# actionml/universal-recommender

Hardware: AMD Instinct MI355X
Metric: cooccurrence pairs/sec (A'A+A'B) + LLR top-k items/sec (higher is better)
Workload: dtype int32 counts / f64 LLR; 1 GPU; config4: synthetic 10M users x 2M items, Zipf-1.0, 5 event types (purchase/view/add-to-cart/search/category-pref); generator=torch Philox on the GPU (universal_recommender_amd.synth.generate_device), maxEventsPerEventType=500, maxCorrelatorsPerEventType=50, seed=20260925, entry_point=urcco_context_build_device (C ABI, include/urcco.h), launch=one process per GPU, parallelism=items range-partitioned over 1 GPU(s), one HIP stream per event type

## Files before the change

universal-recommender_amd/csrc/cco_common.h:

```cpp
#pragma once
#include "cco_kernels.h"

namespace urcco {


constexpr int WAVE = 64;

__device__ __forceinline__ unsigned long long shfl_xor_u64(unsigned long long v, int m) {
  unsigned lo = (unsigned)v, hi = (unsigned)(v >> 32);
  lo = __shfl_xor(lo, m);
  hi = __shfl_xor(hi, m);
  return ((unsigned long long)hi << 32) | lo;
}
__device__ __forceinline__ long long shfl_i64(long long v, int src) {
  unsigned lo = (unsigned)v, hi = (unsigned)((unsigned long long)v >> 32);
  lo = __shfl(lo, src);
  hi = __shfl(hi, src);
  return (long long)(((unsigned long long)hi << 32) | lo);
}
__device__ __forceinline__ long long shfl_up_i64(long long v, unsigned d) {
  unsigned lo = (unsigned)v, hi = (unsigned)((unsigned long long)v >> 32);
  lo = __shfl_up(lo, d);
  hi = __shfl_up(hi, d);
  return (long long)(((unsigned long long)hi << 32) | lo);
// ... 59 lines not shown
    tot += sw;
  }
  __syncthreads();
  *total = tot;
  return base + inc - v;
}

template <typename Load>
__global__ __launch_bounds__(SCAN_THREADS) void scan_reduce_kernel(Load ld, int64_t n, int64_t* __restrict__ tile_sums,
                                                                   const int64_t* __restrict__ n_live) {
  __shared__ long long s_wave[SCAN_THREADS / WAVE];
  const int64_t base = (int64_t)blockIdx.x * SCAN_TILE;
  if (n_live && base >= *n_live) {
    if (threadIdx.x == 0) tile_sums[blockIdx.x] = 0;
    return;
  }
  long long v = 0;
#pragma unroll
  for (int q = 0; q < SCAN_ITEMS; ++q) {
    const int64_t i = base + (int64_t)q * SCAN_THREADS + threadIdx.x;
    if (i < n) v += ld(i);
  }
  long long tot;
  block_exclusive_scan(v, s_wave, &tot);
  if (threadIdx.x == 0) tile_sums[blockIdx.x] = tot;
}

constexpr int ST_THREADS = 1024;
constexpr int ST_ITEMS = 8;
static __global__ __launch_bounds__(ST_THREADS) void scan_tiles_kernel(int64_t* __restrict__ tile_sums, int64_t n_tiles, const int64_t* __restrict__ n_live,
                                                                       ExpandForm form) {
  __shared__ long long s_wave[ST_THREADS / WAVE];
  __shared__ int s_over;
  if (threadIdx.x == 0) s_over = 0;
  __syncthreads();
  bool over = false;
  const int lane = threadIdx.x & (WAVE - 1), wave = threadIdx.x / WAVE;
  int64_t live_tiles = n_tiles;
  if (n_live) {
    const int64_t lt = *n_live / SCAN_TILE + 1;
    if (lt < live_tiles) live_tiles = lt;
  }
  long long carry = form.seed;
  for (int64_t base = 0; base < live_tiles; base += ST_THREADS * ST_ITEMS) {
    const int64_t first = base + (int64_t)threadIdx.x * ST_ITEMS;
    long long x[ST_ITEMS];
    long long sum = 0;
#pragma unroll
    for (int q = 0; q < ST_ITEMS; ++q) {
      x[q] = first + q < live_tiles ? tile_sums[first + q] : 0;
      sum += x[q];
      over = over || (unsigned long long)x[q] >= form.limit;
    }
    long long inc = sum;
#pragma unroll
    for (int d = 1; d < WAVE; d <<= 1) {
      const long long o = shfl_up_i64(inc, d);
      if (lane >= d) inc += o;
    }
    if (lane == WAVE - 1) s_wave[wave] = inc;
    __syncthreads();
    long long before = 0, tot = 0;
#pragma unroll
    for (int w = 0; w < ST_THREADS / WAVE; ++w) {
      const long long sw = s_wave[w];
      if (w < wave) before += sw;
      tot += sw;
    }
    __syncthreads();
    long long run = carry + before + inc - sum;
#pragma unroll
    for (int q = 0; q < ST_ITEMS; ++q) {
      if (first + q < live_tiles) tile_sums[first + q] = run;
      run += x[q];
    }
    carry += tot;
  }
  for (int64_t t = live_tiles + threadIdx.x; t < n_tiles; t += ST_THREADS) tile_sums[t] = carry;
  if (threadIdx.x == 0) tile_sums[n_tiles] = carry;
  if (form.word) {
    if (over) s_over = 1;
    __syncthreads();
    if (threadIdx.x == 0) {
      int f = form.host_narrow ? 0 : *form.word;
      if (form.host_narrow) s_over = 0;
      if (s_over) f |= FORM_TILE;
      if (form.pack_bad && *form.pack_bad != 0) f |= FORM_PACK;
      if (form.host_wide) f |= FORM_HOST;
      *form.word = f ? (f | FORM_WIDE) : 0;
    }
  }
}

template <typename Load>
__global__ __launch_bounds__(SCAN_THREADS) void scan_downsweep_kernel(Load ld, int64_t n, const int64_t* __restrict__ tile_sums,
                                                                      int64_t n_tiles, int64_t* __restrict__ out,
                                                                      const int64_t* __restrict__ n_live) {
  __shared__ long long s_wave[SCAN_THREADS / WAVE];
  if (n_live && (int64_t)blockIdx.x * SCAN_TILE > *n_live) return;
  const int64_t first = (int64_t)blockIdx.x * SCAN_TILE + (int64_t)threadIdx.x * SCAN_ITEMS;
  static_assert(SCAN_ITEMS == 8, "load8");
  long long x[SCAN_ITEMS];
  long long v = 0;
  const bool interior = first + SCAN_ITEMS <= n;
  if (interior) {
    ld.load8(first, x);
  } else {
#pragma unroll
    for (int q = 0; q < SCAN_ITEMS; ++q) x[q] = first + q < n ? ld(first + q) : 0;
  }
#pragma unroll
  for (int q = 0; q < SCAN_ITEMS; ++q) v += x[q];
  long long tot;
  long long run = block_exclusive_scan(v, s_wave, &tot) + tile_sums[blockIdx.x];
  if (interior && (reinterpret_cast<uintptr_t>(out) & 15) == 0) {
#pragma unroll
    for (int q = 0; q < SCAN_ITEMS; q += 2) {
      const long long e0 = run, e1 = run + x[q];
      run = e1 + x[q + 1];
      int4 w;
      w.x = (int)(unsigned)e0; w.y = (int)(unsigned)((unsigned long long)e0 >> 32);
      w.z = (int)(unsigned)e1; w.w = (int)(unsigned)((unsigned long long)e1 >> 32);
      *reinterpret_cast<int4*>(out + first + q) = w;
    }
  } else {
#pragma unroll
    for (int q = 0; q < SCAN_ITEMS; ++q) {
      const int64_t i = first + q;
      if (i < n) out[i] = run;
      run += x[q];
    }
  }
  if (blockIdx.x == 0 && threadIdx.x == 0) out[n] = tile_sums[n_tiles];
}

constexpr int SB_THREADS = 1024;
constexpr int SB_ITEMS = 8;
constexpr int64_t SB_MAX = 32768;
template <typename Load>
__global__ __launch_bounds__(SB_THREADS) void scan_block_kernel(Load ld, int64_t n, int64_t* __restrict__ out) {
  __shared__ long long s_wave[SB_THREADS / WAVE];
  const int lane = threadIdx.x & (WAVE - 1), wave = threadIdx.x / WAVE;
  long long carry = 0;
  for (int64_t base = 0; base < n; base += SB_THREADS * SB_ITEMS) {
    const int64_t first = base + (int64_t)threadIdx.x * SB_ITEMS;
    long long x[SB_ITEMS];
    long long sum = 0;
    if (first + SB_ITEMS <= n) {
      ld.load8(first, x);
    } else {
#pragma unroll
      for (int q = 0; q < SB_ITEMS; ++q) x[q] = first + q < n ? ld(first + q) : 0;
    }
#pragma unroll
    for (int q = 0; q < SB_ITEMS; ++q) sum += x[q];
    long long inc = sum;
#pragma unroll
    for (int d = 1; d < WAVE; d <<= 1) {
      const long long o = shfl_up_i64(inc, d);
      if (lane >= d) inc += o;
    }
    if (lane == WAVE - 1) s_wave[wave] = inc;
    __syncthreads();
    long long before = 0, tot = 0;
#pragma unroll
    for (int w = 0; w < SB_THREADS / WAVE; ++w) {
      const long long sw = s_wave[w];
// ... 30 lines not shown
```

universal-recommender_amd/csrc/cco_counts.hip:

```cpp
#include "cco_kernels.h"

#include <atomic>
#include <cstdio>
#include <cstdlib>

#include "cco_common.h"
#include "cco_device.h"


namespace urcco {

constexpr int CC_THREADS = 256;
constexpr int CC_SLOTS = 4096;

__device__ __forceinline__ void cc_insert(int* s_key, int* s_cnt, int32_t* __restrict__ counts, int col) {
  const int key = col + 1;
  unsigned h = ((unsigned)key * 0x9E3779B1u) >> 20;
#pragma unroll
  for (int probe = 0; probe < 2; ++probe) {
    int kk = __hip_atomic_load(&s_key[h], __ATOMIC_RELAXED, __HIP_MEMORY_SCOPE_WORKGROUP);
    if (kk == 0) kk = atomicCAS(&s_key[h], 0, key), kk = (kk == 0) ? key : kk;
    if (kk == key) {
      atomicAdd(&s_cnt[h], 1);
      return;
// ... 164 lines not shown
    const long long dst = s_base[b];
    for (int t = lane; t < len; t += WAVE) bucketed[dst + t] = s_stage[l0 + t];
  }
}

__global__ __launch_bounds__(SCAN_THREADS) void ph_blockmap_kernel(const int64_t* __restrict__ offsets, int n_buckets, int64_t n_parts,
                                                                  int32_t* __restrict__ blk_prefix, int PH_CHUNK) {
  __shared__ long long s_wave[SCAN_THREADS / WAVE];
  long long carry = 0;
  for (int base = 0; base < n_buckets; base += SCAN_THREADS) {
    const int b = base + threadIdx.x;
    long long v = 0;
    if (b < n_buckets) {
      const long long size = offsets[(int64_t)(b + 1) * n_parts] - offsets[(int64_t)b * n_parts];
      v = (size + PH_CHUNK - 1) / PH_CHUNK;
    }
    long long tot;
    const long long ex = block_exclusive_scan(v, s_wave, &tot);
    if (b < n_buckets) blk_prefix[b] = (int32_t)(carry + ex);
    carry += tot;
  }
  if (threadIdx.x == 0) blk_prefix[n_buckets] = (int32_t)carry;
}

constexpr int PHH_THREADS = 1024;
__global__ __launch_bounds__(PHH_THREADS) void ph_hist_kernel(const unsigned short* __restrict__ bucketed, const int64_t* __restrict__ offsets,
                                                      int n_buckets, int64_t n_parts, const int32_t* __restrict__ blk_prefix,
                                                      unsigned short* __restrict__ partial, int PH_CHUNK) {
  __shared__ unsigned s_cnt[PH_BUCKET];
  const int blk = blockIdx.x;
  if (blk >= blk_prefix[n_buckets]) return;
  int lo = 0, hi = n_buckets;
  while (hi - lo > 1) {
    const int mid = (lo + hi) >> 1;
    if (blk_prefix[mid] <= blk) lo = mid; else hi = mid;
  }
  const int b = lo;
  for (int c = threadIdx.x; c < PH_BUCKET; c += PHH_THREADS) s_cnt[c] = 0u;
  __syncthreads();
  const int64_t bs = offsets[(int64_t)b * n_parts], be = offsets[(int64_t)(b + 1) * n_parts];
  const int64_t e0 = bs + (int64_t)(blk - blk_prefix[b]) * PH_CHUNK;
  const int64_t e1 = e0 + PH_CHUNK < be ? e0 + PH_CHUNK : be;
  int64_t e = e0 + threadIdx.x;
  const int64_t a0 = (e0 + 7) & ~(int64_t)7;
  for (; e < e1 && e < a0; e += PHH_THREADS) atomicAdd(&s_cnt[bucketed[e]], 1u);
  for (int64_t v = a0 + (int64_t)threadIdx.x * 8; v + 7 < e1; v += PHH_THREADS * 8) {
    const uint4 x = *reinterpret_cast<const uint4*>(bucketed + v);
    atomicAdd(&s_cnt[x.x & 0xffffu], 1u); atomicAdd(&s_cnt[x.x >> 16], 1u);
    atomicAdd(&s_cnt[x.y & 0xffffu], 1u); atomicAdd(&s_cnt[x.y >> 16], 1u);
    atomicAdd(&s_cnt[x.z & 0xffffu], 1u); atomicAdd(&s_cnt[x.z >> 16], 1u);
    atomicAdd(&s_cnt[x.w & 0xffffu], 1u); atomicAdd(&s_cnt[x.w >> 16], 1u);
  }
  {
    const int64_t n_vec = e1 > a0 ? (e1 - a0) / 8 : 0;
    for (int64_t t = a0 + n_vec * 8 + threadIdx.x; t < e1; t += PHH_THREADS) atomicAdd(&s_cnt[bucketed[t]], 1u);
  }
  __syncthreads();
  unsigned* out = reinterpret_cast<unsigned*>(partial + (int64_t)blk * PH_BUCKET);
  for (int c = threadIdx.x; c < PH_BUCKET / 2; c += PHH_THREADS) out[c] = s_cnt[2 * c] | (s_cnt[2 * c + 1] << 16);
}

__global__ __launch_bounds__(256) void ph_reduce_kernel(const unsigned short* __restrict__ partial, const int32_t* __restrict__ blk_prefix, int32_t n_cols,
                                                        int32_t* __restrict__ counts) {
  const int64_t j = (int64_t)blockIdx.x * 256 + threadIdx.x;
  if (j >= n_cols) return;
  const int b = (int)(j >> PH_BITS);
  const int c = (int)(j & (PH_BUCKET - 1));
  unsigned sum = 0;
  for (int blk = blk_prefix[b]; blk < blk_prefix[b + 1]; ++blk) sum += partial[(int64_t)blk * PH_BUCKET + c];
  counts[j] = (int32_t)sum;
}

constexpr int PL_BITS = 14;
constexpr int PL_BUCKET = 1 << PL_BITS;
constexpr int PL_PART = 16384;
constexpr int PL_THREADS = 512;
constexpr int PL_PER_THREAD = PL_PART / PL_THREADS;
constexpr int PL_MAX_BUCKETS = 256;
constexpr int PL_COPIES = 16;
static_assert(PL_PER_THREAD % 4 == 0 && PL_PART / PL_COPIES <= 1024 && PL_THREADS % PL_COPIES == 0, "packed word: 8 + 14 + 10 bits");

__global__ __launch_bounds__(PL_THREADS, 6) void pl_partition_kernel(const int32_t* __restrict__ ci, int64_t nnz_host, const int64_t* __restrict__ nnz_dev,
                                                                  int n_buckets, int64_t n_parts, unsigned short* __restrict__ bucketed,
                                                                  unsigned short* __restrict__ loc_t, int vec_ok) {
  __shared__ int s_cnt[PL_COPIES * PL_MAX_BUCKETS];
  __shared__ uint4 s_stage4[PL_PART / 8];
  __shared__ long long s_wave[PL_THREADS / WAVE];
  unsigned short* s_stage = reinterpret_cast<unsigned short*>(s_stage4);
  const int64_t nnz = nnz_dev ? *nnz_dev : nnz_host;
  const int64_t e0 = (int64_t)blockIdx.x * PL_PART;
  const int64_t e1 = e0 + PL_PART < nnz ? e0 + PL_PART : nnz;
  if (e0 >= e1) {
    for (int b = threadIdx.x; b <= n_buckets; b += PL_THREADS) loc_t[(int64_t)b * n_parts + blockIdx.x] = 0;
    return;
  }
  for (int b = threadIdx.x; b < PL_COPIES * n_buckets; b += PL_THREADS) s_cnt[b] = 0;
  __syncthreads();
  int* mine = s_cnt + (threadIdx.x & (PL_COPIES - 1)) * n_buckets;
  const int n = (int)(e1 - e0);
  auto live = [&](int q) { return (q >> 2) * (PL_THREADS * 4) + (int)threadIdx.x * 4 + (q & 3) < n; };
  unsigned w[PL_PER_THREAD];
#pragma unroll
  for (int r = 0; r < PL_PER_THREAD / 4; ++r) {
    const int64_t e = e0 + (int64_t)r * (PL_THREADS * 4) + (int64_t)threadIdx.x * 4;
    int4 x = make_int4(0, 0, 0, 0);
    if (vec_ok && e + 3 < e1) {
      x = *reinterpret_cast<const int4*>(ci + e);
    } else {
      if (e < e1) x.x = ci[e];
      if (e + 1 < e1) x.y = ci[e + 1];
      if (e + 2 < e1) x.z = ci[e + 2];
      if (e + 3 < e1) x.w = ci[e + 3];
    }
    w[4 * r] = (unsigned)x.x; w[4 * r + 1] = (unsigned)x.y; w[4 * r + 2] = (unsigned)x.z; w[4 * r + 3] = (unsigned)x.w;
  }
#pragma unroll
  for (int q = 0; q < PL_PER_THREAD; ++q) {
    if (live(q)) {
      const unsigned b = w[q] >> PL_BITS;
      const unsigned rank = (unsigned)atomicAdd(&mine[b], 1);
      w[q] = (b << 24) | ((w[q] & (PL_BUCKET - 1)) << 10) | rank;
    }
  }
  __syncthreads();
  {
    const int b = threadIdx.x;
    long long tot = 0;
    if (b < n_buckets) {
#pragma unroll
      for (int k = 0; k < PL_COPIES; ++k) tot += s_cnt[k * n_buckets + b];
    }
    long long all;
    const long long ex = block_exclusive_scan<PL_THREADS>(tot, s_wave, &all);
    if (b < n_buckets) {
      int run = (int)ex;
      loc_t[(int64_t)b * n_parts + blockIdx.x] = (unsigned short)run;
#pragma unroll
      for (int k = 0; k < PL_COPIES; ++k) {
        const int c = s_cnt[k * n_buckets + b];
        s_cnt[k * n_buckets + b] = run;
        run += c;
      }
    }
    if (b == n_buckets) loc_t[(int64_t)b * n_parts + blockIdx.x] = (unsigned short)all;
  }
  __syncthreads();
#pragma unroll
  for (int q = 0; q < PL_PER_THREAD; ++q) {
    if (live(q)) s_stage[mine[w[q] >> 24] + (int)(w[q] & 1023u)] = (unsigned short)((w[q] >> 10) & (PL_BUCKET - 1));
  }
  __syncthreads();
  uint4* dst = reinterpret_cast<uint4*>(bucketed + e0);
  for (int v = threadIdx.x; v * 8 < n; v += PL_THREADS) dst[v] = s_stage4[v];
}

constexpr int PLH_THREADS = 1024;
constexpr int PL_LANES = 8;
__global__ __launch_bounds__(PLH_THREADS) void pl_hist_kernel(const unsigned short* __restrict__ bucketed, const unsigned short* __restrict__ loc_t,
                                                              int n_buckets, int64_t n_parts, const int32_t* __restrict__ blk_prefix, int32_t n_cols,
                                                              unsigned* __restrict__ partial) {
  __shared__ unsigned s_cnt[PL_BUCKET];
  const int blk = blockIdx.x;
  if (blk >= blk_prefix[n_buckets]) return;
  int blo = 0, bhi = n_buckets;
  while (bhi - blo > 1) {
    const int mid = (blo + bhi) >> 1;
    if (blk_prefix[mid] <= blk) blo = mid; else bhi = mid;
  }
  const int b = blo, s = blk - blk_prefix[b], S = blk_prefix[b + 1] - blk_prefix[b];
  const int width = (int)((int64_t)n_cols - ((int64_t)b << PL_BITS) < PL_BUCKET ? (int64_t)n_cols - ((int64_t)b << PL_BITS) : PL_BUCKET);
  for (int c = threadIdx.x; c < width; c += PLH_THREADS) s_cnt[c] = 0u;
  __syncthreads();
  const int64_t pp = (n_parts + S - 1) / S;
  const int64_t p0 = (int64_t)s * pp < n_parts ? (int64_t)s * pp : n_parts, p1 = p0 + pp < n_parts ? p0 + pp : n_parts;
  const int lane = threadIdx.x & (WAVE - 1), wave = threadIdx.x / WAVE;
  const unsigned short* lo_t = loc_t + (int64_t)b * n_parts;
  const unsigned short* hi_t = loc_t + (int64_t)(b + 1) * n_parts;
  constexpr int SPR = WAVE / PL_LANES;
  constexpr int GP = 16;
  static_assert(GP % SPR == 0 && SPR <= GP, "rounds per group");
  const int sub = lane / PL_LANES, sl = lane % PL_LANES;
  const int64_t gstep = (int64_t)(PLH_THREADS / WAVE) * GP;
  int64_t g = p0 + (int64_t)wave * GP;
  unsigned lo_n = 0u, hi_n = 0u;
  if (g < p1 && lane < GP && g + lane < p1) {
    lo_n = lo_t[g + lane];
    hi_n = hi_t[g + lane];
  }
  for (; g < p1; g += gstep) {
    const unsigned lo = lo_n, hi = hi_n;
    lo_n = 0u;
    hi_n = 0u;
    if (g + gstep < p1 && lane < GP && g + gstep + lane < p1) {
      lo_n = lo_t[g + gstep + lane];
      hi_n = hi_t[g + gstep + lane];
    }
    const int rounds = (int)(p1 - g < GP ? (p1 - g + SPR - 1) / SPR : GP / SPR);
    for (int r = 0; r < rounds; ++r) {
      const int pj = SPR * r + sub;
      const unsigned lo_j = (unsigned)__shfl((int)lo, pj);
      const unsigned hi_j = (unsigned)__shfl((int)hi, pj);
      const unsigned short* src = bucketed + (g + pj) * PL_PART;
      for (unsigned base = (lo_j & ~7u) + 16u * (unsigned)sl; base < hi_j; base += 16u * PL_LANES) {
        const uint4 x0 = *reinterpret_cast<const uint4*>(src + base), x1 = *reinterpret_cast<const uint4*>(src + base + 8);
        const unsigned wds[8] = {x0.x, x0.y, x0.z, x0.w, x1.x, x1.y, x1.z, x1.w};
#pragma unroll
        for (int k = 0; k < 8; ++k) {
          const unsigned t = base + 2u * k;
          if (t >= lo_j && t < hi_j) atomicAdd(&s_cnt[wds[k] & (PL_BUCKET - 1)], 1u);
          if (t + 1u >= lo_j && t + 1u < hi_j) atomicAdd(&s_cnt[(wds[k] >> 16) & (PL_BUCKET - 1)], 1u);
        }
      }
    }
  }
  __syncthreads();
  unsigned* out = partial + (int64_t)blk * PL_BUCKET;
  for (int c = threadIdx.x; c < width; c += PLH_THREADS) out[c] = s_cnt[c];
}

__global__ __launch_bounds__(256) void pl_reduce_kernel(const unsigned* __restrict__ partial, const int32_t* __restrict__ blk_prefix, int32_t n_cols,
                                                        int32_t* __restrict__ counts) {
  const int64_t j = (int64_t)blockIdx.x * 256 + threadIdx.x;
  if (j >= n_cols) return;
  const int b = (int)(j >> PL_BITS);
  const int c = (int)(j & (PL_BUCKET - 1));
  unsigned sum = 0;
  for (int blk = blk_prefix[b]; blk < blk_prefix[b + 1]; ++blk) sum += partial[(int64_t)blk * PL_BUCKET + c];
  counts[j] = (int32_t)sum;
}

__global__ __launch_bounds__(256) void pl_weights_kernel(const unsigned short* __restrict__ loc_t, int64_t n_parts, unsigned long long* __restrict__ weight) {
  __shared__ long long s_wave[256 / WAVE];
  const unsigned short* lo_t = loc_t + (int64_t)blockIdx.x * n_parts;
  const unsigned short* hi_t = lo_t + n_parts;
  long long sum = 0;
  for (int64_t p = (int64_t)blockIdx.y * 256 + threadIdx.x; p < n_parts; p += (int64_t)gridDim.y * 256) sum += (long long)hi_t[p] - (long long)lo_t[p];
  long long tot;
  block_exclusive_scan<256>(sum, s_wave, &tot);
  if (threadIdx.x == 0 && tot != 0) atomicAdd(&weight[blockIdx.x], (unsigned long long)tot);
}
__global__ __launch_bounds__(SCAN_THREADS) void pl_blockmap_kernel(const long long* __restrict__ weight, int n_buckets, int64_t n_parts, int S,
                                                                  int32_t* __restrict__ blk_prefix) {
  __shared__ long long s_wave[SCAN_THREADS / WAVE];
  __shared__ long long s_total;
  {
    const int b = threadIdx.x;
    long long tot;
    block_exclusive_scan(b < n_buckets ? weight[b] : 0ll, s_wave, &tot);
    if (threadIdx.x == 0) s_total = tot;
  }
  __syncthreads();
  const long long total = s_total;
  const int b = threadIdx.x;
  long long v = 0;
  if (b < n_buckets) {
    v = total > 0 ? (weight[b] * (long long)S * n_buckets + total - 1) / total : 1;
    if (v < 1) v = 1;
    if (v > n_parts) v = n_parts;
  }
  long long tot;
  const long long ex = block_exclusive_scan(v, s_wave, &tot);
  if (b < n_buckets) blk_prefix[b] = (int32_t)ex;
  if (b == 0) blk_prefix[n_buckets] = (int32_t)tot;
}

constexpr int64_t PL_BLOCK_IDS = 49152;
static inline int pl_splits(int n_buckets, int64_t n_parts, bool bounded = true) {
  int64_t S = (2048 + n_buckets - 1) / n_buckets;
  if (S > n_parts / 4) S = n_parts / 4;
  if (bounded) {
    const int64_t by_work = n_parts * PL_PART / ((int64_t)n_buckets * PL_BLOCK_IDS);
    if (S > by_work) S = by_work;
  }
  if (S < 1) S = 1;
  return (int)S;
}
static inline int64_t pl_max_blocks(int n_buckets, int S) { return ((int64_t)S + 1) * n_buckets; }
static inline bool pl_fits(int32_t n_cols) { return (((int64_t)n_cols + PL_BUCKET - 1) >> PL_BITS) <= PL_MAX_BUCKETS; }
static inline bool pl_applies(int32_t n_cols) {
  const char* e = getenv("URCCO_COLCOUNT_GLOBAL_LAYOUT");
  if (e && *e == '1') return false;
  return pl_fits(n_cols);
}

hipError_t launch_slice_weights(hipStream_t st, const unsigned short* loc_t, int n_buckets, int64_t n_parts, long long* weight) {
  hipError_t we = hipMemsetAsync(weight, 0, sizeof(long long) * (size_t)n_buckets, st);
  if (we != hipSuccess) return we;
  const unsigned wsplit = (unsigned)(n_parts >= 8192 ? 8 : (n_parts >= 1024 ? 4 : 1));
  hipLaunchKernelGGL(pl_weights_kernel, dim3((unsigned)n_buckets, wsplit), dim3(256), 0, st, loc_t, n_parts, reinterpret_cast<unsigned long long*>(weight));
  return hipGetLastError();
}

int64_t column_counts_scratch_bytes(int64_t nnz, int32_t n_cols) {
  auto al = [](int64_t v) { return (v + 255) / 256 * 256; };
  if (nnz < PH_MIN_NNZ) return 0;
  int64_t need = 0;
  if (pl_fits(n_cols)) {
    const int64_t n_buckets = ((int64_t)n_cols + PL_BUCKET - 1) >> PL_BITS;
    const int64_t n_parts = (nnz + PL_PART - 1) / PL_PART;
    need = al(n_parts * PL_PART * 2 + 64) + al((n_buckets + 1) * n_parts * 2) + al(n_buckets * 8) + al((n_buckets + 1) * 4) +
           al(pl_max_blocks((int)n_buckets, pl_splits((int)n_buckets, n_parts, false)) * (int64_t)PL_BUCKET * 4);
  }
  if ((((int64_t)n_cols + PH_BUCKET - 1) >> PH_BITS) <= PH_MAX_BUCKETS) {
    const int64_t n_buckets = ((int64_t)n_cols + PH_BUCKET - 1) >> PH_BITS;
    const int64_t n_parts = (nnz + PH_PART - 1) / PH_PART;
    const int64_t m = n_buckets * n_parts;
    const int64_t max_blocks = n_buckets + (nnz + PH_CHUNK_SMALL - 1) / PH_CHUNK_SMALL;
    const int64_t ph = al(m * 4) + al((m + 1) * 8) + al(((m + SCAN_TILE - 1) / SCAN_TILE + 2) * 8) + al(nnz * 2 + 16) + al((n_buckets + 1) * 4) + al(max_blocks * PH_BUCKET * 2);
    if (ph > need) need = ph;
  }
  return need;
}

hipError_t launch_column_counts_partitioned(hipStream_t st, const int32_t* col_idx, int64_t nnz, const int64_t* nnz_dev, int32_t n_cols,
                                            int32_t* counts, char* scratch) {
  auto al = [](int64_t v) { return (v + 255) / 256 * 256; };
  const int vec_ok = (reinterpret_cast<uintptr_t>(col_idx) & 15) == 0;
  if (pl_applies(n_cols)) {
    const int n_buckets = (int)(((int64_t)n_cols + PL_BUCKET - 1) >> PL_BITS);
    const int64_t n_parts = (nnz + PL_PART - 1) / PL_PART;
    const int S = pl_splits(n_buckets, n_parts);
    unsigned short* bucketed = reinterpret_cast<unsigned short*>(scratch); scratch += al(n_parts * PL_PART * 2 + 64);
    unsigned short* loc_t = reinterpret_cast<unsigned short*>(scratch); scratch += al(((int64_t)n_buckets + 1) * n_parts * 2);
    long long* weight = reinterpret_cast<long long*>(scratch); scratch += al((int64_t)n_buckets * 8);
    int32_t* blk_prefix = reinterpret_cast<int32_t*>(scratch); scratch += al(((int64_t)n_buckets + 1) * 4);
    unsigned* partial = reinterpret_cast<unsigned*>(scratch);
    hipLaunchKernelGGL(pl_partition_kernel, dim3((unsigned)n_parts), dim3(PL_THREADS), 0, st, col_idx, nnz, nnz_dev, n_buckets, n_parts, bucketed, loc_t, vec_ok);
    hipError_t we = launch_slice_weights(st, loc_t, n_buckets, n_parts, weight);
    if (we != hipSuccess) return we;
    hipLaunchKernelGGL(pl_blockmap_kernel, dim3(1), dim3(SCAN_THREADS), 0, st, weight, n_buckets, n_parts, S, blk_prefix);
    hipLaunchKernelGGL(pl_hist_kernel, dim3((unsigned)pl_max_blocks(n_buckets, S)), dim3(PLH_THREADS), 0, st, bucketed, loc_t, n_buckets, n_parts,
                       blk_prefix, n_cols, partial);
    hipLaunchKernelGGL(pl_reduce_kernel, dim3((unsigned)(((int64_t)n_cols + 255) / 256)), dim3(256), 0, st, partial, blk_prefix, n_cols, counts);
    return hipGetLastError();
  }
  const int n_buckets = (int)(((int64_t)n_cols + PH_BUCKET - 1) >> PH_BITS);
  const int64_t n_parts = (nnz + PH_PART - 1) / PH_PART;
  const int64_t m = (int64_t)n_buckets * n_parts;
  const int chunk = ph_chunk(nnz);
  const int64_t max_blocks = n_buckets + (nnz + chunk - 1) / chunk;
  int32_t* part_counts = reinterpret_cast<int32_t*>(scratch); scratch += al(m * 4);
  int64_t* offsets = reinterpret_cast<int64_t*>(scratch); scratch += al((m + 1) * 8);
  int64_t* tile_sums = reinterpret_cast<int64_t*>(scratch); scratch += al(((m + SCAN_TILE - 1) / SCAN_TILE + 2) * 8);
  unsigned short* bucketed = reinterpret_cast<unsigned short*>(scratch); scratch += al(nnz * 2 + 16);
  int32_t* blk_prefix = reinterpret_cast<int32_t*>(scratch); scratch += al(((int64_t)n_buckets + 1) * 4);
  unsigned short* partial = reinterpret_cast<unsigned short*>(scratch);
  hipLaunchKernelGGL(ph_count_kernel, dim3((unsigned)n_parts), dim3(256), 0, st, col_idx, nnz, nnz_dev, n_buckets, n_parts, part_counts, vec_ok);
  hipError_t e = launch_scan_i32(st, part_counts, m, offsets, tile_sums);
  if (e != hipSuccess) return e;
  hipLaunchKernelGGL(ph_scatter_kernel, dim3((unsigned)n_parts), dim3(PHS_THREADS), 0, st, col_idx, nnz, nnz_dev, n_buckets, n_parts, offsets, bucketed, vec_ok);
  hipLaunchKernelGGL(ph_blockmap_kernel, dim3(1), dim3(SCAN_THREADS), 0, st, offsets, n_buckets, n_parts, blk_prefix, chunk);
  hipLaunchKernelGGL(ph_hist_kernel, dim3((unsigned)max_blocks), dim3(PHH_THREADS), 0, st, bucketed, offsets, n_buckets, n_parts, blk_prefix, partial, chunk);
  hipLaunchKernelGGL(ph_reduce_kernel, dim3((unsigned)(((int64_t)n_cols + 255) / 256)), dim3(256), 0, st, partial, blk_prefix, n_cols, counts);
  return hipGetLastError();
}

struct PopBounds { long long b[4]; };
__global__ __launch_bounds__(CC_THREADS) void pop_counts_kernel(int64_t n, const int32_t* __restrict__ item, const int64_t* __restrict__ t_ms,
                                                              int32_t n_items, int n_buckets, PopBounds bounds, int32_t* __restrict__ counts) {
  __shared__ int s_key[CC_SLOTS];
  __shared__ int s_cnt[CC_SLOTS];
  for (int s = threadIdx.x; s < CC_SLOTS; s += CC_THREADS) {
    s_key[s] = 0;
    s_cnt[s] = 0;
  }
  __syncthreads();
  for (int64_t e = (int64_t)blockIdx.x * CC_THREADS + threadIdx.x; e < n; e += (int64_t)gridDim.x * CC_THREADS) {
    const int i = item[e];
    if (i < 0 || i >= n_items) continue;
    const long long t = t_ms[e];
    int b = -1;
#pragma unroll
    for (int k = 0; k < 3; ++k)
      if (k < n_buckets && t >= bounds.b[k] && t < bounds.b[k + 1]) b = k;
    if (b >= 0) cc_insert(s_key, s_cnt, counts, b * n_items + i);
  }
  __syncthreads();
  for (int s = threadIdx.x; s < CC_SLOTS; s += CC_THREADS)
    if (s_key[s] != 0) atomicAdd(&counts[s_key[s] - 1], s_cnt[s]);
}
hipError_t launch_pop_counts(hipStream_t st, int n_cu, int64_t n, const int32_t* item, const int64_t* t_ms, int32_t n_items, int n_buckets,
                             const int64_t* bounds, int32_t* counts) {
  hipError_t e = hipMemsetAsync(counts, 0, sizeof(int32_t) * (size_t)n_items * (size_t)n_buckets, st);
  if (e != hipSuccess || n == 0) return e;
  PopBounds pb;
  for (int k = 0; k < 4; ++k) pb.b[k] = k <= n_buckets ? bounds[k] : bounds[n_buckets];
  int64_t blocks = (n + (int64_t)CC_THREADS * 8 - 1) / ((int64_t)CC_THREADS * 8);
  const int64_t cap = (int64_t)n_cu * 4;
  if (blocks > cap) blocks = cap;
  if (blocks < 1) blocks = 1;
  hipLaunchKernelGGL(pop_counts_kernel, dim3((unsigned)blocks), dim3(CC_THREADS), 0, st, n, item, t_ms, n_items, n_buckets, pb, counts);
  return hipGetLastError();
}


}
```

universal-recommender_amd/csrc/cco_expand.hip:

```cpp
#include "cco_kernels.h"

#include <atomic>
#include <cstdio>
#include <cstdlib>

#include "cco_common.h"
#include "cco_device.h"


namespace urcco {

__global__ __launch_bounds__(256) void item_entropy_kernel(const int32_t* __restrict__ counts, int32_t n, long long n_users,
                                                           double* __restrict__ ent, double* __restrict__ xlx_n) {
  const int64_t i = (int64_t)blockIdx.x * 256 + threadIdx.x;
  if (i < n) {
    const long long c = counts[i];
    ent[i] = entropy2(c, n_users - c);
  }
  if (i == 0 && xlx_n) *xlx_n = x_log_x(n_users);
}

hipError_t launch_item_entropy(hipStream_t st, const int32_t* counts, int32_t n, long long n_users, double* ent, double* xlx_n) {
  const int blocks = n > 0 ? (n + 255) / 256 : 1;
  hipLaunchKernelGGL(item_entropy_kernel, dim3(blocks), dim3(256), 0, st, counts, n, n_users, ent, xlx_n);
  return hipGetLastError();
}

__global__ __launch_bounds__(256) void narrow_counts_kernel(const int32_t* __restrict__ counts, int64_t n, unsigned short* __restrict__ out16,
                                                            int32_t* __restrict__ bad) {
  int over = 0;
  for (int64_t i = (int64_t)blockIdx.x * 256 + threadIdx.x; i < n; i += (int64_t)gridDim.x * 256) {
    const int c = counts[i];
    out16[i] = (unsigned short)c;
    over += (c < 0 || c > 0xffff) ? 1 : 0;
  }
  if (over) atomicAdd(bad, over);
}
hipError_t launch_narrow_counts(hipStream_t st, int n_cu, const int32_t* counts, int64_t n, unsigned short* out16, int32_t* bad) {
  hipError_t e = hipMemsetAsync(bad, 0, sizeof(int32_t), st);
  if (e != hipSuccess || n <= 0) return e;
  int64_t blocks = (n + 255) / 256;
  if (blocks > (int64_t)n_cu * 8) blocks = (int64_t)n_cu * 8;
  hipLaunchKernelGGL(narrow_counts_kernel, dim3((unsigned)blocks), dim3(256), 0, st, counts, n, out16, bad);
  return hipGetLastError();
}

typedef int urcco_v4i __attribute__((ext_vector_type(4)));
__device__ __forceinline__ int4 nt_load4(const int32_t* p) {
#ifdef HIPSIM_HOST_BUILD
  return *reinterpret_cast<const int4*>(p);
#else
  const urcco_v4i v = __builtin_nontemporal_load(reinterpret_cast<const urcco_v4i*>(p));
  return make_int4(v.x, v.y, v.z, v.w);
#endif
}
__device__ __forceinline__ void nt_store4(int32_t* p, int4 y) {
#ifdef HIPSIM_HOST_BUILD
  *reinterpret_cast<int4*>(p) = y;
#else
  urcco_v4i v;
  v.x = y.x; v.y = y.y; v.z = y.z; v.w = y.w;
  __builtin_nontemporal_store(v, reinterpret_cast<urcco_v4i*>(p));
#endif
}
__global__ __launch_bounds__(256) void pack_counts_kernel(const int32_t* __restrict__ ci, const int64_t* __restrict__ nnz_dev, int64_t nnz_bound,
                                                          const unsigned short* __restrict__ cnt, const int32_t* __restrict__ bad16, int shift,
                                                          int32_t* __restrict__ out, int32_t* __restrict__ bad, int vec_ok) {
  if (*bad16 != 0) {
    if (blockIdx.x == 0 && threadIdx.x == 0) *bad = 1;
    return;
  }
  int64_t nnz = *nnz_dev;
  if (nnz > nnz_bound) nnz = nnz_bound;
  const unsigned limit = 32 - shift >= 16 ? 65536u : (1u << (32 - shift));
  int n_bad = 0;
  const int64_t nvec = vec_ok ? nnz >> 2 : 0;
  const int64_t stride = (int64_t)gridDim.x * 256;
  for (int64_t v = (int64_t)blockIdx.x * 256 + threadIdx.x; v < nvec; v += 2 * stride) {
    const bool two = v + stride < nvec;
    const int4 x = nt_load4(ci + 4 * v);
    const int4 z = two ? nt_load4(ci + 4 * (v + stride)) : make_int4(0, 0, 0, 0);
    const unsigned c0 = (unsigned)cnt[x.x], c1 = (unsigned)cnt[x.y], c2 = (unsigned)cnt[x.z], c3 = (unsigned)cnt[x.w];
    const unsigned d0 = two ? (unsigned)cnt[z.x] : 0u, d1 = two ? (unsigned)cnt[z.y] : 0u, d2 = two ? (unsigned)cnt[z.z] : 0u, d3 = two ? (unsigned)cnt[z.w] : 0u;
    n_bad += (c0 >= limit) + (c1 >= limit) + (c2 >= limit) + (c3 >= limit) + (d0 >= limit) + (d1 >= limit) + (d2 >= limit) + (d3 >= limit);
    int4 y;
    y.x = (int)((unsigned)x.x | (c0 << shift)); y.y = (int)((unsigned)x.y | (c1 << shift));
    y.z = (int)((unsigned)x.z | (c2 << shift)); y.w = (int)((unsigned)x.w | (c3 << shift));
    nt_store4(out + 4 * v, y);
    if (two) {
      y.x = (int)((unsigned)z.x | (d0 << shift)); y.y = (int)((unsigned)z.y | (d1 << shift));
      y.z = (int)((unsigned)z.z | (d2 << shift)); y.w = (int)((unsigned)z.w | (d3 << shift));
      nt_store4(out + 4 * (v + stride), y);
    }
  }
  for (int64_t e = (nvec << 2) + (int64_t)blockIdx.x * 256 + threadIdx.x; e < nnz; e += stride) {
    const unsigned j = (unsigned)ci[e], c = (unsigned)cnt[j];
    n_bad += c >= limit;
    out[e] = (int)(j | (c << shift));
  }
  if (n_bad) atomicAdd(bad, n_bad);
}
hipError_t launch_pack_counts(hipStream_t st, int n_cu, const int32_t* col_idx, const int64_t* nnz_dev, int64_t nnz_bound, const unsigned short* counts16,
                              const int32_t* bad16, int32_t count_bits, int32_t* out, int32_t* bad) {
  hipError_t e = hipMemsetAsync(bad, 0, sizeof(int32_t), st);
  if (e != hipSuccess || nnz_bound <= 0) return e;
  const int shift = 32 - count_bits;
  int64_t blocks = (nnz_bound / 4 + 255) / 256;
  const int64_t cap = (int64_t)n_cu * 16;
  if (blocks > cap) blocks = cap;
  if (blocks < 1) blocks = 1;
  const int vec_ok = ((reinterpret_cast<uintptr_t>(col_idx) | reinterpret_cast<uintptr_t>(out)) & 15) == 0;
  hipLaunchKernelGGL(pack_counts_kernel, dim3((unsigned)blocks), dim3(256), 0, st, col_idx, nnz_dev, nnz_bound, counts16, bad16, shift, out, bad, vec_ok);
  return hipGetLastError();
}

__global__ __launch_bounds__(256) void xlx_table_kernel(double* __restrict__ tab) {
  const int x = blockIdx.x * 256 + threadIdx.x;
  if (x < XLX_TABLE) tab[x] = x_log_x((long long)x);
}
hipError_t launch_xlx_table(hipStream_t st, double* tab) {
  hipLaunchKernelGGL(xlx_table_kernel, dim3(XLX_TABLE / 256), dim3(256), 0, st, tab);
  return hipGetLastError();
}
__global__ __launch_bounds__(256) void xlx_hi_table_kernel(double* __restrict__ tab, const double* __restrict__ xlx_tab, long long n_users) {
  const int d = blockIdx.x * 256 + threadIdx.x;
  if (d >= XLX_TABLE) return;
  tab[d] = n_users - d >= 0 ? x_log_x(n_users - (long long)d) : 0.0;
  const double hi = n_users - d >= 0 ? x_log_x(n_users - (long long)d) : 0.0;
  tab[XLX_TABLE + d] = d <= n_users ? (x_log_x(n_users) - x_log_x_tab((long long)d, xlx_tab)) - hi : 0.0;
}
hipError_t launch_xlx_hi_table(hipStream_t st, double* tab, const double* xlx_tab, long long n_users) {
  hipLaunchKernelGGL(xlx_hi_table_kernel, dim3(XLX_TABLE / 256), dim3(256), 0, st, tab, xlx_tab, n_users);
  return hipGetLastError();
}

__global__ __launch_bounds__(SCAN_THREADS) void expand_downsweep_kernel(const int32_t* __restrict__ plen, int64_t n, const int64_t* __restrict__ tile_sums,
                                                                        int64_t n_tiles, int64_t* __restrict__ out, const int64_t* __restrict__ n_live,
                                                                        const int32_t* __restrict__ form, const unsigned* __restrict__ pstart32,
                                                                        int64_t* __restrict__ pstart64) {
  __shared__ long long s_wave[SCAN_THREADS / WAVE];
  if ((int64_t)blockIdx.x * SCAN_TILE > *n_live) return;
  const int f = *form;
  const LoadI32 ld{plen};
  const int64_t first = (int64_t)blockIdx.x * SCAN_TILE + (int64_t)threadIdx.x * SCAN_ITEMS;
  static_assert(SCAN_ITEMS == 8, "load8");
  long long x[SCAN_ITEMS];
  long long v = 0;
  const bool interior = first + SCAN_ITEMS <= n;
  if (interior) {
    ld.load8(first, x);
  } else {
#pragma unroll
    for (int q = 0; q < SCAN_ITEMS; ++q) x[q] = first + q < n ? ld(first + q) : 0;
  }
#pragma unroll
  for (int q = 0; q < SCAN_ITEMS; ++q) v += x[q];
  long long tot;
  long long run = block_exclusive_scan(v, s_wave, &tot) + tile_sums[blockIdx.x];
  if (f == 0) {
    unsigned* out32 = reinterpret_cast<unsigned*>(out);
    unsigned r = (unsigned)run;
    if (interior && (reinterpret_cast<uintptr_t>(out) & 15) == 0) {
      unsigned e[SCAN_ITEMS];
#pragma unroll
      for (int q = 0; q < SCAN_ITEMS; ++q) {
        e[q] = r;
        r += (unsigned)x[q];
      }
      *reinterpret_cast<uint4*>(out32 + first) = make_uint4(e[0], e[1], e[2], e[3]);
      *reinterpret_cast<uint4*>(out32 + first + 4) = make_uint4(e[4], e[5], e[6], e[7]);
    } else {
#pragma unroll
      for (int q = 0; q < SCAN_ITEMS; ++q) {
        if (first + q < n) out32[first + q] = r;
        r += (unsigned)x[q];
      }
    }
    if (blockIdx.x == 0 && threadIdx.x == 0) out32[n] = (unsigned)tile_sums[n_tiles];
    return;
  }
  if (interior && (reinterpret_cast<uintptr_t>(out) & 15) == 0) {
#pragma unroll
    for (int q = 0; q < SCAN_ITEMS; q += 2) {
      const long long e0 = run, e1 = run + x[q];
      run = e1 + x[q + 1];
      int4 w;
      w.x = (int)(unsigned)e0; w.y = (int)(unsigned)((unsigned long long)e0 >> 32);
// ... 142 lines not shown
            constexpr int W = 2 * N;
#pragma unroll
            for (int d = 0; d + 4 <= W; d += 4) {
              const Words4 x = *reinterpret_cast<const Words4*>(t + d);
              v[q][d] = x.a; v[q][(d + 1) % W] = x.b; v[q][(d + 2) % W] = x.c; v[q][(d + 3) % W] = x.d;
            }
            if (W % 4 >= 2) {
              const Words2 x = *reinterpret_cast<const Words2*>(t + (W / 4) * 4);
              v[q][(W / 4) * 4 % W] = x.a; v[q][((W / 4) * 4 + 1) % W] = x.b;
            }
            if (W % 2 == 1) v[q][W - 1] = t[W - 1];
          }
        } else {
#pragma unroll
          for (int d = 0; d < 2 * N; ++d) v[q][d] = 0u;
        }
      }
#pragma unroll
      for (int q = 0; q < 2; ++q) {
        const int64_t p = base + (int64_t)(r + q) * 256 + threadIdx.x;
        if (p < lim) {
#pragma unroll
          for (int d = 0; d < N; ++d) {
            const int32_t len = (int32_t)(v[q][N + d] - v[q][d]);
            a.pstart[d][p] = v[q][d];
            a.plen[d][p] = len;
            sum[d] += (long long)len;
          }
        }
      }
    }
#pragma unroll
    for (int d = 0; d < N; ++d) {
      unsigned long long x = (unsigned long long)sum[d];
#pragma unroll
      for (int m = 1; m < WAVE; m <<= 1) x += shfl_xor_u64(x, m);
      if ((threadIdx.x & (WAVE - 1)) == 0) s_part[threadIdx.x / WAVE][d] = (long long)x;
    }
    __syncthreads();
    if (threadIdx.x < N && a.tsum[threadIdx.x]) {
      long long tot = 0;
#pragma unroll
      for (int w = 0; w < 256 / WAVE; ++w) tot += s_part[w][threadIdx.x];
      a.tsum[threadIdx.x][tile] = tot;
    }
    __syncthreads();
  }
}
hipError_t launch_expand_prepare_multi(hipStream_t st, int n_cu, const int64_t* a_col_ptr, int32_t n_items_a, const int32_t* a_row_idx, int n,
                                       const int64_t* const* b_row_ptr, int64_t n_rows_b, int64_t cap, unsigned* const* pstart, int32_t* const* plen, void* T,
                                       int64_t* const* tsum) {
  if (n < 1 || n > EXPAND_MULTI_MAX) return hipErrorInvalidValue;
  if (cap <= 0) return hipSuccess;
  ExpandMultiArgs a;
  a.n = n;
  for (int d = 0; d < EXPAND_MULTI_MAX; ++d) {
    a.b_rp[d] = d < n ? b_row_ptr[d] : nullptr;
    a.pstart[d] = d < n ? pstart[d] : nullptr;
    a.plen[d] = d < n ? plen[d] : nullptr;
    a.tsum[d] = (d < n && tsum) ? tsum[d] : nullptr;
  }
  int64_t nb = (n_rows_b + 255) / 256;
  if (nb > (int64_t)n_cu * 8) nb = (int64_t)n_cu * 8;
  if (nb < 1) nb = 1;
  hipLaunchKernelGGL(expand_pack_kernel, dim3((unsigned)nb), dim3(256), 0, st, a, n_rows_b, static_cast<unsigned*>(T));
  int64_t blocks = (cap + SCAN_TILE - 1) / SCAN_TILE;
  const int64_t lim = (int64_t)n_cu * 16;
  if (blocks > lim) blocks = lim;
  const unsigned* Tc = static_cast<const unsigned*>(T);
  switch (n) {
    case 1: hipLaunchKernelGGL(expand_prepare_multi_kernel<1>, dim3((unsigned)blocks), dim3(256), 0, st, a_col_ptr, n_items_a, a_row_idx, Tc, cap, a); break;
    case 2: hipLaunchKernelGGL(expand_prepare_multi_kernel<2>, dim3((unsigned)blocks), dim3(256), 0, st, a_col_ptr, n_items_a, a_row_idx, Tc, cap, a); break;
    case 3: hipLaunchKernelGGL(expand_prepare_multi_kernel<3>, dim3((unsigned)blocks), dim3(256), 0, st, a_col_ptr, n_items_a, a_row_idx, Tc, cap, a); break;
    case 4: hipLaunchKernelGGL(expand_prepare_multi_kernel<4>, dim3((unsigned)blocks), dim3(256), 0, st, a_col_ptr, n_items_a, a_row_idx, Tc, cap, a); break;
    case 5: hipLaunchKernelGGL(expand_prepare_multi_kernel<5>, dim3((unsigned)blocks), dim3(256), 0, st, a_col_ptr, n_items_a, a_row_idx, Tc, cap, a); break;
    case 6: hipLaunchKernelGGL(expand_prepare_multi_kernel<6>, dim3((unsigned)blocks), dim3(256), 0, st, a_col_ptr, n_items_a, a_row_idx, Tc, cap, a); break;
    case 7: hipLaunchKernelGGL(expand_prepare_multi_kernel<7>, dim3((unsigned)blocks), dim3(256), 0, st, a_col_ptr, n_items_a, a_row_idx, Tc, cap, a); break;
    default: hipLaunchKernelGGL(expand_prepare_multi_kernel<8>, dim3((unsigned)blocks), dim3(256), 0, st, a_col_ptr, n_items_a, a_row_idx, Tc, cap, a); break;
  }
  return hipGetLastError();
}
hipError_t launch_expand_scan(hipStream_t st, const int64_t* a_col_ptr, int32_t n_items_a, const int32_t* plen, int64_t cap, int64_t* wp, int64_t* tile_sums,
                              bool tile_sums_ready, const unsigned* pstart32, int64_t* pstart64, ExpandForm form) {
  hipError_t e = hipMemsetAsync(form.word, 0, sizeof(int32_t), st);
  if (e != hipSuccess) return e;
  return expand_scan(st, plen, cap, wp, tile_sums, a_col_ptr + n_items_a, tile_sums_ready, pstart32, pstart64, form);
}

__device__ __forceinline__ int64_t work_prefix_at(const int64_t* __restrict__ wp, const int64_t* __restrict__ tile_sums, bool narrow, int64_t p) {
  if (!narrow) return wp[p];
  const int64_t base = tile_sums[p / SCAN_TILE];
  return base + (int64_t)(unsigned)(reinterpret_cast<const unsigned*>(wp)[p] - (unsigned)base);
}
__global__ __launch_bounds__(256) void row_work_kernel(int32_t item_lo, int32_t item_hi, const int64_t* __restrict__ a_cp,
                                                       const int64_t* __restrict__ wp, const int64_t* __restrict__ tile_sums, const int32_t* __restrict__ form,
                                                       int64_t* __restrict__ work) {
  const int64_t n = (int64_t)item_hi - item_lo;
  const bool narrow = *form == 0;
  for (int64_t t = (int64_t)blockIdx.x * 256 + threadIdx.x; t < n; t += (int64_t)gridDim.x * 256) {
    const int64_t i = item_lo + t;
    work[t] = work_prefix_at(wp, tile_sums, narrow, a_cp[i + 1]) - work_prefix_at(wp, tile_sums, narrow, a_cp[i]);
  }
}

hipError_t launch_row_work(hipStream_t st, int n_cu, int32_t item_lo, int32_t item_hi, const int64_t* a_col_ptr, const int64_t* wp, const int64_t* tile_sums,
                           const int32_t* form, int64_t* work) {
  const int64_t n = (int64_t)item_hi - item_lo;
  if (n <= 0) return hipSuccess;
  int64_t blocks = (n + 255) / 256;
  const int64_t cap = (int64_t)n_cu * 8;
  if (blocks > cap) blocks = cap;
  hipLaunchKernelGGL(row_work_kernel, dim3((unsigned)blocks), dim3(256), 0, st, item_lo, item_hi, a_col_ptr, wp, tile_sums, form, work);
  return hipGetLastError();
}


}
```

universal-recommender_amd/csrc/cco_kernels.h:

```cpp
#pragma once
#include <hip/hip_runtime.h>
#include <stdint.h>

namespace urcco {

constexpr int NBINS = 7;
constexpr int MP_KMAX_HOST = 256;

constexpr int SCAN_TILE = 2048;
constexpr int DS_TILE = 4096;
constexpr int GLOBAL_BIN_BLOCKS = 128;
constexpr int BIN_TILE = 1024;
constexpr int XLX_TABLE_HOST = 4096;
constexpr int BIN_COLS_HOST = 3 * NBINS + 3;
constexpr int BIN_OFF_LEN = NBINS + 3;
constexpr int CAND_SLOTS = 64;
constexpr int STATS_LEN = 32;

constexpr int32_t DBG_GATHER_ONLY = 1;
constexpr int32_t DBG_NO_LLR = 2;
constexpr int32_t DBG_NO_TOPK = 4;
constexpr int32_t DBG_NO_SELECT = 8;
constexpr int32_t DBG_NO_RANK = 16;
constexpr int32_t DBG_NO_COUNT_GATHER = 512;
constexpr int32_t DBG_UNFUSED_EXPAND = 4096;
constexpr int32_t DBG_GATHERED_PRIMARY = 8192;
constexpr int32_t DBG_UNFILTERED_EXCHANGE = 16384;
constexpr int32_t DBG_SELECT_DELAY = 131072;
constexpr int32_t DBG_UNPACKED_COUNTS = 1048576;
constexpr int32_t DBG_ROW_KERNELS = DBG_GATHER_ONLY | DBG_NO_LLR | DBG_NO_TOPK | DBG_NO_SELECT | DBG_NO_RANK | DBG_NO_COUNT_GATHER | DBG_SELECT_DELAY;

constexpr int32_t FORM_WIDE = 1;
constexpr int32_t FORM_PS64 = 2;
constexpr int32_t FORM_TILE = 4;
constexpr int32_t FORM_PACK = 8;
constexpr int32_t FORM_HOST = 16;
constexpr unsigned long long NARROW_LIMIT = 1ull << 32;
struct ExpandForm {
  int32_t* word;
  const int32_t* pack_bad;
  int32_t host_wide;
  int32_t host_narrow;
  unsigned long long limit;
  long long seed;
};

struct CcoArgs {
  const int32_t* bin_rows;
  const int32_t* bin_off;
  const int64_t* a_col_ptr;
  const unsigned* pstart32;
  const int64_t* wp;
  const int32_t* b_col_idx;
  const int32_t* b_packed;
  const int32_t* form;
  int32_t pk_known;
  uint32_t b_col_mask;
  const int32_t* cnt_a;
  const int32_t* cnt_b;
  const double* ent_a;
  const unsigned short* cnt_b16;
  const int32_t* cnt16_bad;
  const double* xlx_n;
  const double* xlx_tab;
  const double* xlx_hi;
  const double* col_ent;
  int32_t debug;
  long long n_users;
  int32_t n_cols_b;
  int32_t item_lo;
  int32_t exclude_self;
  int32_t k;
  int32_t has_min_llr;
  double min_llr;
  int32_t count_bits;
  int32_t col_bytes;
  int32_t g_log2;
  int32_t unordered;
  int32_t* out_count;
  int32_t* out_idx;
  double* out_llr;
  unsigned long long* err;
  unsigned long long* cand;
  int32_t* g_counts;
  unsigned long long* g_cand_key;
  int32_t* g_cand_col;
  int32_t g_blocks;
  const int64_t* pstart64;
  const int64_t* work;
};

hipError_t launch_column_counts(hipStream_t st, int n_cu, const int32_t* col_idx, int64_t nnz, int32_t n_cols, int32_t* counts);
constexpr int64_t PH_MIN_NNZ = 1 << 20;
int64_t column_counts_scratch_bytes(int64_t nnz, int32_t n_cols);
hipError_t launch_column_counts_partitioned(hipStream_t st, const int32_t* col_idx, int64_t nnz, const int64_t* nnz_dev, int32_t n_cols,
                                            int32_t* counts, char* scratch);

hipError_t launch_scan_i32(hipStream_t st, const int32_t* in, int64_t n, int64_t* out, int64_t* tile_sums);
hipError_t launch_slice_weights(hipStream_t st, const unsigned short* loc_t, int n_buckets, int64_t n_parts, long long* weight);

hipError_t launch_downsample_flags(hipStream_t st, int n_cu, int64_t n_rows, const int64_t* row_ptr, const int32_t* col_idx, int64_t nnz,
                                   int32_t n_cols, const int32_t* raw_counts, unsigned long long* thresholds, uint32_t seed, int32_t max_n,
                                   int row_rate_mode, int64_t row_base, int64_t* tile_rows, unsigned long long* flags, int64_t* tile_count,
                                   int32_t* post_counts);
hipError_t launch_downsample_scan(hipStream_t st, int64_t nnz, int64_t* tile_count);
hipError_t launch_downsample_compact(hipStream_t st, int64_t n_rows, const int64_t* row_ptr, const int32_t* col_idx, int64_t nnz,
                                     const int64_t* tile_rows, const unsigned long long* flags, const int64_t* tile_off, int64_t* out_row_ptr,
                                     int32_t* out_col_idx);

hipError_t launch_scan_i32_range(hipStream_t st, const int32_t* in, int64_t n, int32_t lo, int32_t hi, int64_t* out, int64_t* tile_sums);
hipError_t launch_transpose(hipStream_t st, int n_cu, int64_t n_rows, const int64_t* row_ptr, const int32_t* col_idx, int g_log2,
                            const int64_t* col_ptr, int32_t* cursor, int32_t* out_row_idx, int32_t col_lo, int32_t col_hi);
int64_t transpose_scratch_bytes(int64_t n_rows, int64_t nnz, int32_t n_cols);
hipError_t launch_transpose_partitioned(hipStream_t st, int64_t n_rows, const int64_t* row_ptr, const int32_t* col_idx, int64_t nnz, int32_t n_cols,
                                        const int64_t* col_ptr, int32_t* cursor , int32_t* out_row_idx, int32_t col_lo, int32_t col_hi, char* scratch);
hipError_t launch_row_work_csr(hipStream_t st, int n_cu, int64_t n_rows, const int64_t* a_row_ptr, const int32_t* a_col_idx,
                               const int64_t* b_row_ptr, int g_log2, int32_t n_items_a, int64_t* work);

struct KeyTable {
  unsigned long long* keys;
  unsigned* minpos;
  unsigned* count;
  int32_t* id;
  unsigned long long mask;
};
hipError_t launch_dictionary_build(hipStream_t st, int n_cu, KeyTable t, int64_t n, const unsigned long long* keys, const int32_t* select,
                                   int32_t min_count, int32_t* flag, int64_t* prefix, int64_t* tile_sums, int64_t* first_pos);
hipError_t launch_dictionary_lookup(hipStream_t st, int n_cu, KeyTable t, int64_t n, const unsigned long long* keys, const int32_t* select,
                                    int32_t* ids);
hipError_t launch_dictionary_verify(hipStream_t st, int n_cu, KeyTable t, int64_t n, const unsigned long long* keys, const int32_t* select,
                                    const unsigned long long* check, const unsigned long long* ref_check, const int64_t* first_pos, unsigned long long* err);
hipError_t launch_csr_from_pairs(hipStream_t st, int n_cu, int64_t n, const int32_t* rows, const int32_t* cols, int64_t n_rows, int32_t* cnt,
                                 int64_t* raw_ptr, int32_t* tmp, int64_t* tile_sums, int64_t* out_row_ptr, int32_t* out_col_idx);

constexpr int EXCH_SIZES = 4;
hipError_t launch_row_lengths(hipStream_t st, int n_cu, int64_t n_rows, const int64_t* row_ptr, int32_t* len, unsigned short* len16, int64_t* sizes);
hipError_t launch_counts_over_limit(hipStream_t st, int n_cu, const int32_t* counts, int64_t n, int32_t count_bits, int64_t* out);
hipError_t launch_need_mask(hipStream_t st, int n_cu, int64_t n_rows, const int64_t* a_row_ptr, const int32_t* a_col_idx, const int32_t* bounds, int world,
                            unsigned long long* mask);
hipError_t launch_masked_lengths(hipStream_t st, int n_cu, int64_t n_rows, const int64_t* row_ptr, const unsigned long long* mask, int world, int32_t* mlen, int64_t* off,
                                 int64_t* tile_sums, int64_t* to_nnz);
hipError_t launch_pack_rows(hipStream_t st, int n_cu, int64_t n_rows, const int64_t* row_ptr, const int32_t* col_idx, const unsigned long long* mask, int world,
                            const int64_t* off, int32_t* pack);
hipError_t launch_scan_u16(hipStream_t st, const unsigned short* in, int64_t n, int64_t* out, int64_t* tile_sums);
hipError_t launch_frag_record(hipStream_t st, int32_t world, const int32_t* bounds, const int64_t* l_cp, const int32_t* bad, int64_t* rec);
hipError_t launch_frag_place(hipStream_t st, int n_cu, int32_t world, int32_t lo, int32_t n_range, const void* lens, int wire16, const int64_t* src_off,
                             const int32_t* ents, const int64_t* a_cp, const int64_t* sizes, int32_t* a_ri);

hipError_t launch_validate_csr(hipStream_t st, int n_cu, int64_t n_rows, const int64_t* row_ptr, const int32_t* col_idx, int64_t nnz, int32_t n_cols,
                               int g_log2, int64_t rp0, unsigned long long* err);
hipError_t launch_rebase_i64(hipStream_t st, int n_cu, int64_t* p, int64_t n, int64_t delta);
hipError_t launch_publish_word(hipStream_t st, const unsigned long long* src, unsigned long long* dst_mapped);

hipError_t launch_pop_counts(hipStream_t st, int n_cu, int64_t n, const int32_t* item, const int64_t* t_ms, int32_t n_items, int n_buckets,
                             const int64_t* bounds, int32_t* counts);

hipError_t launch_pack_counts(hipStream_t st, int n_cu, const int32_t* col_idx, const int64_t* nnz_dev, int64_t nnz_bound, const unsigned short* counts16,
                              const int32_t* bad16, int32_t count_bits, int32_t* out, int32_t* bad);
hipError_t launch_xlx_table(hipStream_t st, double* tab);
hipError_t launch_xlx_hi_table(hipStream_t st, double* tab , const double* xlx_tab, long long n_users);
hipError_t launch_item_entropy(hipStream_t st, const int32_t* counts, int32_t n, long long n_users, double* ent, double* xlx_n);
hipError_t launch_narrow_counts(hipStream_t st, int n_cu, const int32_t* counts, int64_t n, unsigned short* out16, int32_t* bad);

hipError_t launch_expand_prepare(hipStream_t st, int n_cu, const int64_t* a_col_ptr, int32_t n_items_a, const int32_t* a_row_idx,
                                 const int64_t* b_row_ptr, unsigned* b_rp32_scratch , int64_t n_rows_b, int64_t cap,
                                 unsigned* pstart32, int64_t* pstart64, int32_t* plen, int64_t* wp, int64_t* tile_sums, ExpandForm form);
constexpr int EXPAND_MULTI_MAX = 8;
hipError_t launch_expand_prepare_multi(hipStream_t st, int n_cu, const int64_t* a_col_ptr, int32_t n_items_a, const int32_t* a_row_idx, int n,
                                       const int64_t* const* b_row_ptr, int64_t n_rows_b, int64_t cap, unsigned* const* pstart, int32_t* const* plen, void* T,
                                       int64_t* const* tsum );
hipError_t launch_expand_scan(hipStream_t st, const int64_t* a_col_ptr, int32_t n_items_a, const int32_t* plen, int64_t cap, int64_t* wp, int64_t* tile_sums,
                              bool tile_sums_ready, const unsigned* pstart32, int64_t* pstart64, ExpandForm form);
hipError_t launch_row_work(hipStream_t st, int n_cu, int32_t item_lo, int32_t item_hi, const int64_t* a_col_ptr, const int64_t* wp, const int64_t* tile_sums,
                           const int32_t* form, int64_t* work);

hipError_t launch_binning(hipStream_t st, int32_t item_lo, int32_t n, const int64_t* work, const int32_t* cnt_a, int32_t n_cols_b,
                          int32_t count_bits, int32_t k, int64_t* tile_counts, int32_t* bin_off, int32_t* bin_rows, int64_t* stats);

hipError_t launch_cco_rows_bin(hipStream_t st, int n_cu, const CcoArgs& args, int bin, int32_t n_rows );
hipError_t launch_bin_out_stats(hipStream_t st, const int32_t* bin_rows, const int32_t* bin_off, int32_t item_lo, const int32_t* out_count,
                                const unsigned long long* cand, int64_t* stats);

hipError_t launch_compact_indicators(hipStream_t st, int32_t n_rows, int32_t k, const int32_t* count, const int32_t* idx,
                                     const double* llr, const int64_t* row_ptr, int32_t* out_idx, double* out_llr);

hipError_t launch_partition(hipStream_t st, int32_t n_items, const int64_t* work_prefix, int32_t n_parts, int32_t* bounds);
hipError_t launch_scan_i64(hipStream_t st, const int64_t* in, int64_t n, int64_t* out, int64_t* tile_sums);

constexpr int REC_MAX_CLAUSES = 16;
constexpr int REC_MAX_NUM = 256;
constexpr int REC_NO_BACKFILL = 1;
constexpr int REC_STATS_LEN = 8;
constexpr int REC_LDS_LIMIT = 3072;
struct RecClause {
  const int64_t* ind_col_ptr;
  const int32_t* ind_row_idx;
  const int64_t* q_row_ptr;
  const int32_t* q_col_idx;
  double boost;
  int32_t n_cols;
  int32_t reserved;
};
constexpr int REC_MAX_RULES = 16;
constexpr int REC_RULE_ANY = 0;
constexpr int REC_RULE_NONE = 1;
constexpr int REC_RULE_RANGE = 2;
struct RecRule {
  const int64_t* m_row_ptr;
  const int32_t* m_col_idx;
  const int64_t* q_row_ptr;
  const int32_t* q_col_idx;
  const int64_t* item_value;
  const int64_t* q_lo;
  const int64_t* q_hi;
  int32_t kind, n_cols;
};
struct RecArgs;
int32_t recommend_global_blocks(int64_t n_queries, int32_t n_items, int n_cu);
hipError_t launch_recommend(hipStream_t st, int n_cu, int64_t n_queries, int32_t n_items, const RecClause* clauses, int32_t n_clauses, const int64_t* excl_row_ptr,
                            const int32_t* excl_col_idx, const uint8_t* item_mask, const int32_t* fill_order, int32_t num, int32_t flags, int32_t* out_count,
                            int32_t* out_idx, double* out_score, int64_t* stats_dev, unsigned long long* ctr, int32_t* list, int32_t* pos, int32_t g_blocks,
                            unsigned* g_state, unsigned* g_m, int32_t* g_list, double* g_score, int32_t lds_limit = REC_LDS_LIMIT, const RecRule* rules = nullptr,
                            int32_t n_rules = 0);

hipError_t launch_llr_test(hipStream_t st, int64_t n, const int64_t* a, const int64_t* b, const int64_t* ab, const int64_t* nu, double* out);
hipError_t launch_u01_test(hipStream_t st, int64_t n, uint32_t seed, const int32_t* row, const int32_t* col, double* out, int rng32 = 0);

}
```

universal-recommender_amd/csrc/cco_rows.hip:

```cpp
#include "cco_kernels.h"

#include <atomic>
#include <cstdlib>

#include "cco_common.h"
#include "cco_device.h"


namespace urcco {

constexpr int E0 = 1024, E1S = 4096, E1 = 8192, E2S = 16384, E2 = 32768;
constexpr int MP_KMAX = 256;

__host__ __device__ constexpr int table_slots(int E, int T) { return (2 * E / 3) / (2 * T) * (2 * T); }
constexpr int URCCO_WB1 = 512;
constexpr int URCCO_WB2 = 8192;
__device__ __forceinline__ int choose_bin(long long w, long long ca, int32_t n_cols_b, int32_t count_bits, int32_t k) {
  if (ca <= 0 || w <= 0) return -1;
  if (count_bits < 31 && ca > ((1ll << count_bits) - 1)) return NBINS - 1;
  if (w <= 64 && ca <= 64) return 0;
  int cap_bin = NBINS - 1;
  const long long dmax = (w < (long long)n_cols_b ? w : (long long)n_cols_b) * 3 + (long long)k * 3 + 2;
  if (dmax <= E0) cap_bin = 1;
  else if (dmax <= E1S) cap_bin = 2;
// ... 48 lines not shown
      for (int k = 0; k < IBINS; ++k) c[k] += (ib == k);
#pragma unroll
      for (int k = 0; k < NBINS; ++k) {
        pw[k] += (b == k) ? w : 0;
        pu[k] += (b == k) ? ca : 0;
      }
    }
  }
#pragma unroll
  for (int k = 0; k < IBINS; ++k)
    if (c[k]) atomicAdd((unsigned long long*)&s_acc[k], (unsigned long long)c[k]);
#pragma unroll
  for (int k = 0; k < NBINS; ++k)
    if (pu[k]) {
      atomicAdd((unsigned long long*)&s_acc[IBINS + k], (unsigned long long)pw[k]);
      atomicAdd((unsigned long long*)&s_acc[IBINS + NBINS + k], (unsigned long long)pu[k]);
    }
  if (pairs) atomicAdd((unsigned long long*)&s_acc[IBINS + 2 * NBINS], (unsigned long long)pairs);
  __syncthreads();
  if (threadIdx.x < BIN_COLS) tile_counts[(int64_t)blockIdx.x * BIN_COLS + threadIdx.x] = s_acc[threadIdx.x];
}

constexpr int BS_THREADS = 1024;
__global__ __launch_bounds__(BS_THREADS) void bin_scan_kernel(int64_t* __restrict__ tile_counts, int64_t n_tiles, int32_t* __restrict__ bin_off,
                                                              int64_t* __restrict__ stats) {
  __shared__ long long s_tot[BIN_COLS];
  const int lane = threadIdx.x & (WAVE - 1), wave = threadIdx.x / WAVE;
  for (int k = wave; k < BIN_COLS; k += BS_THREADS / WAVE) {
    if (k >= IBINS) {
      long long acc = 0;
      for (int64_t base = 0; base < n_tiles; base += 4 * WAVE) {
        long long v[4];
#pragma unroll
        for (int q = 0; q < 4; ++q) {
          const int64_t i = base + q * WAVE + lane;
          v[q] = i < n_tiles ? tile_counts[i * BIN_COLS + k] : 0;
        }
        acc += (v[0] + v[1]) + (v[2] + v[3]);
      }
#pragma unroll
      for (int d = 1; d < WAVE; d <<= 1) {
        const long long o = shfl_up_i64(acc, d);
        if (lane >= d) acc += o;
      }
      acc = shfl_i64(acc, WAVE - 1);
      if (lane == 0) s_tot[k] = acc;
      continue;
    }
    long long carry = 0;
    for (int64_t base = 0; base < n_tiles; base += WAVE) {
      const int64_t i = base + lane;
      const long long v = i < n_tiles ? tile_counts[i * BIN_COLS + k] : 0;
      long long inc = v;
#pragma unroll
      for (int d = 1; d < WAVE; d <<= 1) {
        const long long o = shfl_up_i64(inc, d);
        if (lane >= d) inc += o;
      }
      if (i < n_tiles) tile_counts[i * BIN_COLS + k] = carry + inc - v;
      carry += shfl_i64(inc, WAVE - 1);
    }
    if (lane == 0) s_tot[k] = carry;
  }
  __syncthreads();
  if (threadIdx.x == 0) {
    int32_t off = 0;
    for (int ib = 0; ib < IBINS; ++ib) {
      if (ib == 0) bin_off[0] = off;
      else if (ib < MICRO_SUBS) bin_off[NBINS + ib] = off;
      else bin_off[ib - (MICRO_SUBS - 1)] = off;
      off += (int32_t)s_tot[ib];
    }
    bin_off[NBINS] = off;
    if (stats) {
      for (int k = 0; k < NBINS; ++k) {
        long long rows = 0;
        if (k == 0) for (int q = 0; q < MICRO_SUBS; ++q) rows += s_tot[q];
        else rows = s_tot[k + MICRO_SUBS - 1];
        stats[1 + k] = rows;
        stats[1 + NBINS + k] = s_tot[IBINS + k];
        stats[1 + 2 * NBINS + k] = s_tot[IBINS + NBINS + k];
      }
      stats[0] = s_tot[IBINS + 2 * NBINS];
      stats[STATS_LEN - 1] = s_tot[0] + s_tot[1];
    }
  }
}

__global__ __launch_bounds__(BIN_THREADS) void bin_scatter_kernel(int32_t item_lo, int32_t n, const int64_t* __restrict__ work,
                                                                  const int32_t* __restrict__ cnt_a, int32_t n_cols_b, int32_t count_bits, int32_t k,
                                                                  const int64_t* __restrict__ tile_counts, const int32_t* __restrict__ bin_off,
                                                                  int32_t* __restrict__ bin_rows, int split) {
  __shared__ long long s_wave[SCAN_THREADS / WAVE];
  int b[BIN_ITEMS];
#pragma unroll
  for (int q = 0; q < BIN_ITEMS; ++q) {
    const int64_t t = (int64_t)blockIdx.x * BIN_TILE + (int64_t)threadIdx.x * BIN_ITEMS + q;
    b[q] = -1;
    if (t < n) {
      const long long w = work[t], ca = cnt_a[item_lo + t];
      b[q] = internal_bin(choose_bin(w, ca, n_cols_b, count_bits, k), w, ca, split);
    }
  }
  for (int k = 0; k < IBINS; ++k) {
    int c = 0;
#pragma unroll
    for (int q = 0; q < BIN_ITEMS; ++q) c += (b[q] == k);
    long long tot;
    long long pos = block_exclusive_scan(c, s_wave, &tot) + tile_counts[(int64_t)blockIdx.x * BIN_COLS + k] + internal_start(bin_off, k);
#pragma unroll
    for (int q = 0; q < BIN_ITEMS; ++q)
      if (b[q] == k) bin_rows[pos++] = item_lo + (int32_t)((int64_t)blockIdx.x * BIN_TILE + (int64_t)threadIdx.x * BIN_ITEMS + q);
  }
}

hipError_t launch_binning(hipStream_t st, int32_t item_lo, int32_t n, const int64_t* work, const int32_t* cnt_a, int32_t n_cols_b,
                          int32_t count_bits, int32_t k, int64_t* tile_counts, int32_t* bin_off, int32_t* bin_rows, int64_t* stats) {
  if (n <= 0) {
    hipError_t e = hipMemsetAsync(bin_off, 0, sizeof(int32_t) * BIN_OFF_LEN, st);
    if (e == hipSuccess && stats) e = hipMemsetAsync(stats, 0, sizeof(int64_t) * STATS_LEN, st);
    return e;
  }
  const int64_t n_tiles = ((int64_t)n + BIN_TILE - 1) / BIN_TILE;
  const int split = micro_split_for(n) ? 1 : 0;
  hipLaunchKernelGGL(bin_count_kernel, dim3((unsigned)n_tiles), dim3(BIN_THREADS), 0, st, item_lo, n, work, cnt_a, n_cols_b, count_bits, k, tile_counts, split);
  hipLaunchKernelGGL(bin_scan_kernel, dim3(1), dim3(BS_THREADS), 0, st, tile_counts, n_tiles, bin_off, stats);
  hipLaunchKernelGGL(bin_scatter_kernel, dim3((unsigned)n_tiles), dim3(BIN_THREADS), 0, st, item_lo, n, work, cnt_a, n_cols_b, count_bits, k,
                     tile_counts, bin_off, bin_rows, split);
  return hipGetLastError();
}

struct Best {
  unsigned long long key;
  int col;
};
__device__ __forceinline__ bool best_before(unsigned long long ka, int ca, unsigned long long kb, int cb) {
  return ka > kb || (ka == kb && ca < cb);
}

__device__ __forceinline__ bool llr_operands_in_tables(unsigned k11, long long ca, unsigned cb, long long n_users, const double* col_ent) {
  const long long k12 = ca - (long long)k11, k21 = (long long)cb - (long long)k11, d22 = ca + k21;
  return col_ent != nullptr && (unsigned long long)(k12 | k21 | (long long)cb | d22) < (unsigned long long)XLX_TABLE && d22 <= n_users;
}
__device__ __forceinline__ double llr_from_tables(double row_entropy, double xlx_n, unsigned k11, unsigned ca, unsigned cb, const double* __restrict__ xlx_tab,
                                                  const double* __restrict__ xlx_hi, const double* __restrict__ col_ent) {
  double t11 = xlx_tab[k11], t12 = xlx_tab[ca - k11], t21 = xlx_tab[cb - k11], t22 = xlx_hi[ca + cb - k11], tce = col_ent[cb];
#ifndef HIPSIM_HOST_BUILD
  asm volatile("" : "+v"(t11), "+v"(t12), "+v"(t21), "+v"(t22), "+v"(tce));
#endif
  const double matrix_entropy = (((xlx_n - t11) - t12) - t21) - t22;
  const double s = row_entropy + tce;
  if (s < matrix_entropy) return 0.0;
  return 2.0 * (s - matrix_entropy);
}
__device__ __forceinline__ double llr_of(double row_entropy, double xlx_n, long long k11, long long ca, long long cb, long long n_users,
                                         const double* __restrict__ xlx_tab, const double* __restrict__ xlx_hi, const double* __restrict__ col_ent) {
  return llr_from_entropies_tab(row_entropy, column_entropy_of(cb, xlx_n, n_users, xlx_tab, xlx_hi, col_ent), xlx_n, k11, ca - k11, cb - k11, n_users - ca - cb + k11, xlx_tab,
                                n_users, xlx_hi);
}

__device__ __forceinline__ void count_if_before(unsigned& r, unsigned long long ka, unsigned ca, unsigned long long mk, unsigned mc) {
#ifdef HIPSIM_HOST_BUILD
  r += best_before(ka, (int)ca, mk, (int)mc) ? 1u : 0u;
#else
  unsigned t;
  asm("v_sub_co_u32 %1, vcc, %2, %3\n\t"
// ... 1461 lines not shown
```

universal-recommender_amd/csrc/cco_transpose.hip:

```cpp
#include "cco_kernels.h"

#include <atomic>
#include <cstdio>
#include <cstdlib>

#include "cco_common.h"
#include "cco_device.h"


namespace urcco {

__global__ __launch_bounds__(256) void transpose_kernel(int64_t n_rows, const int64_t* __restrict__ rp, const int32_t* __restrict__ ci,
                                                        int g_log2, const int64_t* __restrict__ col_ptr, int32_t* __restrict__ cursor,
                                                        int32_t* __restrict__ out_rows, int32_t col_lo, int32_t col_hi) {
  const int G = 1 << g_log2;
  const int gl = threadIdx.x & (G - 1);
  const int64_t groups_per_block = 256 >> g_log2;
  for (int64_t r = (int64_t)blockIdx.x * groups_per_block + (threadIdx.x >> g_log2); r < n_rows;
       r += (int64_t)gridDim.x * groups_per_block) {
    const int64_t s = rp[r], e = rp[r + 1];
    for (int64_t p = s + gl; p < e; p += G) {
      const int j = ci[p];
      if (j < col_lo || j >= col_hi) continue;
      const int pos = atomicAdd(&cursor[j], 1);
      out_rows[col_ptr[j] + pos] = (int32_t)r;
    }
  }
}

hipError_t launch_transpose(hipStream_t st, int n_cu, int64_t n_rows, const int64_t* row_ptr, const int32_t* col_idx, int g_log2,
                            const int64_t* col_ptr, int32_t* cursor, int32_t* out_row_idx, int32_t col_lo, int32_t col_hi) {
  if (n_rows == 0) return hipSuccess;
  const int64_t gpb = 256 >> g_log2;
  int64_t blocks = (n_rows + gpb - 1) / gpb;
  const int64_t cap = (int64_t)n_cu * 8;
  if (blocks > cap) blocks = cap;
  hipLaunchKernelGGL(transpose_kernel, dim3((unsigned)blocks), dim3(256), 0, st, n_rows, row_ptr, col_idx, g_log2, col_ptr, cursor, out_row_idx, col_lo,
                     col_hi);
  return hipGetLastError();
}

constexpr int TR_PART = 16384;
constexpr int64_t TR_CHUNK = 1 << 18;

__global__ __launch_bounds__(256) void tr_parts_kernel(int64_t n_rows, const int64_t* __restrict__ rp, int64_t n_parts, int64_t* __restrict__ R) {
  const int64_t p = (int64_t)blockIdx.x * 256 + threadIdx.x;
  if (p > n_parts) return;
  if (p == n_parts) { R[p] = n_rows; return; }
  const int64_t target = p * TR_PART;
  int64_t lo = 0, hi = n_rows;
  while (lo < hi) {
    const int64_t mid = lo + ((hi - lo) >> 1);
    if (rp[mid] >= target) hi = mid; else lo = mid + 1;
  }
  R[p] = lo;
}

constexpr int TP_PART = TR_PART;
constexpr int TP_THREADS = 512;
constexpr int TP_PER_THREAD = TP_PART / TP_THREADS;
constexpr int TP_COPIES = 4;
constexpr int TP_MAX_BUCKETS = 512;
constexpr int TP_MAX_BITS = 14;
constexpr int TP_WORDS = TP_PART / 64;
static_assert(TP_PER_THREAD % 4 == 0 && TP_MAX_BUCKETS <= TP_THREADS && TP_WORDS <= TP_THREADS, "one scan round; one thread per mask word");

static int tp_bucket_bits(int32_t n_cols) {
  int bits = 6;
  while (bits < TP_MAX_BITS && (((int64_t)n_cols + ((int64_t)1 << bits) - 1) >> bits) > TP_MAX_BUCKETS) ++bits;
  return bits;
}

__global__ __launch_bounds__(TP_THREADS, 4) void tp_partition_kernel(int64_t n_rows, const int64_t* __restrict__ rp, const int32_t* __restrict__ ci,
                                                                  const int64_t* __restrict__ R, int bits, int n_buckets, int64_t n_parts, int32_t col_lo,
                                                                  int32_t col_hi, unsigned short* __restrict__ bk_col, unsigned short* __restrict__ bk_row16,
                                                                  int32_t* __restrict__ bk_row, int64_t* __restrict__ part_base,
                                                                  unsigned short* __restrict__ loc_t, int vec_ok) {
  __shared__ int s_cnt[TP_COPIES * TP_MAX_BUCKETS];
  __shared__ uint4 s_stage4[TP_PART / 8];
  __shared__ unsigned long long s_mask[TP_WORDS];
  __shared__ __attribute__((aligned(16))) unsigned short s_row_at[TP_PART];
  __shared__ int s_tbefore[TP_WORDS];
  __shared__ long long s_wave[TP_THREADS / WAVE];
  __shared__ int s_wmax[TP_WORDS / WAVE];
  unsigned short* s_stage = reinterpret_cast<unsigned short*>(s_stage4);
  const int64_t part = blockIdx.x;
  const int64_t nnz = rp[n_rows];
  const int64_t e0 = part * TP_PART;
  if (e0 >= nnz) {
    for (int b = threadIdx.x; b <= n_buckets; b += TP_THREADS) loc_t[(int64_t)b * n_parts + part] = 0;
    if (threadIdx.x == 0) part_base[part] = 0;
    return;
  }
  const int n = (int)(e0 + TP_PART < nnz ? TP_PART : nnz - e0);
  int cols[TP_PER_THREAD];
#pragma unroll
  for (int r = 0; r < TP_PER_THREAD / 4; ++r) {
    const int el0 = r * (TP_THREADS * 4) + (int)threadIdx.x * 4;
    const int64_t e = e0 + el0;
    int4 x = make_int4(-1, -1, -1, -1);
    if (vec_ok && el0 + 3 < n) {
      x = *reinterpret_cast<const int4*>(ci + e);
    } else {
      if (el0 < n) x.x = ci[e];
      if (el0 + 1 < n) x.y = ci[e + 1];
      if (el0 + 2 < n) x.z = ci[e + 2];
      if (el0 + 3 < n) x.w = ci[e + 3];
    }
    cols[4 * r] = x.x; cols[4 * r + 1] = x.y; cols[4 * r + 2] = x.z; cols[4 * r + 3] = x.w;
  }
  for (int b = threadIdx.x; b < TP_COPIES * n_buckets; b += TP_THREADS) s_cnt[b] = 0;
  if (threadIdx.x < TP_WORDS) s_mask[threadIdx.x] = 0ull;
  const int64_t g0 = R[part];
  const int64_t r_s = (g0 < n_rows && rp[g0] == e0) ? g0 : g0 - 1;
  const int64_t g1 = R[part + 1];
  const int64_t r_e = g1 < n_rows ? g1 : n_rows;
  const int64_t n_slice = r_e - r_s + 1;
  const bool by_marks = n_slice <= 65536;
  __syncthreads();
  if (by_marks) {
    for (int64_t t = threadIdx.x; t + 1 < n_slice; t += TP_THREADS) {
      const int64_t a = rp[r_s + t] - e0, b = rp[r_s + t + 1] - e0;
      if (b > a && a >= 0) {
        s_row_at[a] = (unsigned short)t;
        atomicOr(&s_mask[a >> 6], 1ull << (a & 63));
      }
    }
  }
// ... 36 lines not shown
  }
  __syncthreads();
  {
    const int b = threadIdx.x;
    long long tot = 0;
    if (b < n_buckets) {
#pragma unroll
      for (int k = 0; k < TP_COPIES; ++k) tot += s_cnt[k * n_buckets + b];
    }
    long long all;
    const long long ex = block_exclusive_scan<TP_THREADS>(tot, s_wave, &all);
    if (b < n_buckets) {
      int run = (int)ex;
      loc_t[(int64_t)b * n_parts + part] = (unsigned short)run;
#pragma unroll
      for (int k = 0; k < TP_COPIES; ++k) {
        const int c = s_cnt[k * n_buckets + b];
        s_cnt[k * n_buckets + b] = run;
        run += c;
      }
    }
    if (b == n_buckets % TP_THREADS) loc_t[(int64_t)n_buckets * n_parts + part] = (unsigned short)all;
  }
  __syncthreads();
  const unsigned cmask = (1u << bits) - 1u;
  if (by_marks) {
    unsigned t2[TP_PER_THREAD / 2];
#pragma unroll
    for (int r = 0; r < TP_PER_THREAD / 4; ++r) {
      const int el0 = r * (TP_THREADS * 4) + (int)threadIdx.x * 4;
      const int w = el0 >> 6, sh = el0 & 63;
      const unsigned long long m = s_mask[w];
      const unsigned starts = (unsigned)(m >> sh) & 0xfu;
      const unsigned long long low = m & ((1ull << sh) - 1ull);
      unsigned t_cur = (unsigned)s_tbefore[w];
      if (low) t_cur = (unsigned)s_row_at[w * 64 + 63 - __clzll((long long)low)];
      const uint2 at2 = *reinterpret_cast<const uint2*>(&s_row_at[el0]);
      const unsigned at[4] = {at2.x & 0xffffu, at2.x >> 16, at2.y & 0xffffu, at2.y >> 16};
      unsigned tq[4];
#pragma unroll
      for (int q = 0; q < 4; ++q) {
        t_cur = (starts >> q) & 1u ? at[q] : t_cur;
        tq[q] = t_cur;
      }
      t2[2 * r] = tq[0] | (tq[1] << 16);
      t2[2 * r + 1] = tq[2] | (tq[3] << 16);
    }
    __syncthreads();
#pragma unroll
    for (int q = 0; q < TP_PER_THREAD; ++q) {
      const int j = cols[q];
      if (j >= 0) {
        const unsigned rk = (q & 1) ? rank2[q >> 1] >> 16 : rank2[q >> 1] & 0xffffu;
        const int pos = mine[j >> bits] + (int)rk;
        s_stage[pos] = (unsigned short)((unsigned)j & cmask);
        s_row_at[pos] = (unsigned short)((q & 1) ? t2[q >> 1] >> 16 : t2[q >> 1] & 0xffffu);
      }
    }
    __syncthreads();
    uint4* rdst = reinterpret_cast<uint4*>(bk_row16 + e0);
    const uint4* rsrc = reinterpret_cast<const uint4*>(s_row_at);
    for (int v = threadIdx.x; v * 8 < n; v += TP_THREADS) rdst[v] = rsrc[v];
    if (threadIdx.x == 0) part_base[part] = r_s;
  } else {
    int32_t* row_dst = bk_row + e0;
#pragma unroll 1
    for (int q = 0; q < TP_PER_THREAD; ++q) {
      const int j = cols[q];
      if (j >= 0) {
        const int el = (q >> 2) * (TP_THREADS * 4) + (int)threadIdx.x * 4 + (q & 3);
        const unsigned rk = (q & 1) ? rank2[q >> 1] >> 16 : rank2[q >> 1] & 0xffffu;
        const int pos = mine[j >> bits] + (int)rk;
        s_stage[pos] = (unsigned short)((unsigned)j & cmask);
        row_dst[pos] = (int)(upper_bound_i64(rp, r_s, r_e, e0 + el) - 1);
      }
    }
    __syncthreads();
    if (threadIdx.x == 0) part_base[part] = -1;
  }
  uint4* dst = reinterpret_cast<uint4*>(bk_col + e0);
  for (int v = threadIdx.x; v * 8 < n; v += TP_THREADS) dst[v] = s_stage4[v];
}

__global__ __launch_bounds__(SCAN_THREADS) void tp_blockmap_kernel(const long long* __restrict__ weight, int n_buckets, int64_t n_parts, int32_t* __restrict__ blk_prefix) {
  __shared__ long long s_wave[SCAN_THREADS / WAVE];
  long long carry = 0;
  for (int base = 0; base < n_buckets; base += SCAN_THREADS) {
    const int b = base + threadIdx.x;
    long long v = 0;
    if (b < n_buckets) {
      v = weight[b] > 0 ? (weight[b] + TR_CHUNK - 1) / TR_CHUNK : 1;
      if (v > n_parts) v = n_parts;
    }
    long long tot;
    const long long ex = block_exclusive_scan(v, s_wave, &tot);
    if (b < n_buckets) blk_prefix[b] = (int32_t)(carry + ex);
    carry += tot;
  }
  if (threadIdx.x == 0) blk_prefix[n_buckets] = (int32_t)carry;
}

constexpr int TPP_THREADS = 1024;
constexpr int TPP_LPS = 4;
__global__ __launch_bounds__(TPP_THREADS) void tp_place_kernel(const unsigned short* __restrict__ bk_col, const unsigned short* __restrict__ bk_row16,
                                                               const int32_t* __restrict__ bk_row, const int64_t* __restrict__ part_base,
                                                               const unsigned short* __restrict__ loc_t, int bits, int n_buckets, int64_t n_parts,
                                                               const int32_t* __restrict__ blk_prefix, const int64_t* __restrict__ col_ptr, int32_t n_cols,
                                                               int32_t* __restrict__ g_cursor , int32_t* __restrict__ out_rows) {
  __shared__ unsigned s_cur[1 << TP_MAX_BITS];
  const int blk = blockIdx.x;
  if (blk >= blk_prefix[n_buckets]) return;
  int blo = 0, bhi = n_buckets;
  while (bhi - blo > 1) {
    const int mid = (blo + bhi) >> 1;
    if (blk_prefix[mid] <= blk) blo = mid; else bhi = mid;
  }
  const int b = blo, s = blk - blk_prefix[b], S = blk_prefix[b + 1] - blk_prefix[b];
  const int width = 1 << bits;
  const int64_t col0 = (int64_t)b << bits;
  const bool shared_cursors = S > 1;
  const int64_t base = col_ptr[col0];
  if (!shared_cursors) {
    for (int c = threadIdx.x; c < width; c += TPP_THREADS) s_cur[c] = col0 + c < n_cols ? (unsigned)(col_ptr[col0 + c] - base) : 0u;
  }
  __syncthreads();
  const int64_t pp = (n_parts + S - 1) / S;
  const int64_t p0 = (int64_t)s * pp < n_parts ? (int64_t)s * pp : n_parts, p1 = p0 + pp < n_parts ? p0 + pp : n_parts;
  const int lane = threadIdx.x & (WAVE - 1), wave = threadIdx.x / WAVE;
  const unsigned short* lo_t = loc_t + (int64_t)b * n_parts;
  const unsigned short* hi_t = loc_t + (int64_t)(b + 1) * n_parts;
  constexpr int GP = WAVE / TPP_LPS;
  const int sub = lane / TPP_LPS, sl = lane % TPP_LPS;
  const int64_t gstep = (int64_t)(TPP_THREADS / WAVE) * GP;
  int64_t g = p0 + (int64_t)wave * GP;
  unsigned lo_n = 0u, hi_n = 0u;
  int pb_n = 0;
  if (g < p1 && lane < GP && g + lane < p1) {
    lo_n = lo_t[g + lane];
    hi_n = hi_t[g + lane];
    pb_n = (int)part_base[g + lane];
  }
  for (; g < p1; g += gstep) {
    const unsigned lo = lo_n, hi = hi_n;
    const int pb = pb_n;
    lo_n = 0u;
    hi_n = 0u;
    pb_n = 0;
    if (g + gstep < p1 && lane < GP && g + gstep + lane < p1) {
      lo_n = lo_t[g + gstep + lane];
      hi_n = hi_t[g + gstep + lane];
      pb_n = (int)part_base[g + gstep + lane];
    }
    const unsigned lo_j = (unsigned)__shfl((int)lo, sub);
    const unsigned hi_j = (unsigned)__shfl((int)hi, sub);
    const int pb_j = __shfl(pb, sub);
    const unsigned short* csrc = bk_col + (g + sub) * TP_PART;
    const unsigned short* r16 = bk_row16 + (g + sub) * TP_PART;
    const int32_t* rsrc = bk_row + (g + sub) * TP_PART;
    for (unsigned at = (lo_j & ~7u) + 8u * (unsigned)sl; at < hi_j; at += 8u * TPP_LPS) {
      const uint4 c4 = *reinterpret_cast<const uint4*>(csrc + at);
      int rr[8];
      if (pb_j >= 0) {
        const uint4 t4 = *reinterpret_cast<const uint4*>(r16 + at);
        rr[0] = pb_j + (int)(t4.x & 0xffffu); rr[1] = pb_j + (int)(t4.x >> 16); rr[2] = pb_j + (int)(t4.y & 0xffffu); rr[3] = pb_j + (int)(t4.y >> 16);
        rr[4] = pb_j + (int)(t4.z & 0xffffu); rr[5] = pb_j + (int)(t4.z >> 16); rr[6] = pb_j + (int)(t4.w & 0xffffu); rr[7] = pb_j + (int)(t4.w >> 16);
      } else {
        const int4 r0 = *reinterpret_cast<const int4*>(rsrc + at), r1 = *reinterpret_cast<const int4*>(rsrc + at + 4);
        rr[0] = r0.x; rr[1] = r0.y; rr[2] = r0.z; rr[3] = r0.w; rr[4] = r1.x; rr[5] = r1.y; rr[6] = r1.z; rr[7] = r1.w;
      }
      const unsigned cw[4] = {c4.x, c4.y, c4.z, c4.w};
#pragma unroll
      for (int k = 0; k < 8; ++k) {
        const unsigned t = at + (unsigned)k;
        if (t >= lo_j && t < hi_j) {
          const unsigned c = (k & 1) ? cw[k >> 1] >> 16 : cw[k >> 1] & 0xffffu;
          if (shared_cursors) out_rows[col_ptr[col0 + c] + atomicAdd(&g_cursor[col0 + c], 1)] = rr[k];
          else out_rows[base + atomicAdd(&s_cur[c], 1u)] = rr[k];
        }
      }
    }
  }
}

static void tp_geometry(int64_t nnz, int32_t n_cols, int* bits, int64_t* n_buckets, int64_t* n_parts) {
  *bits = tp_bucket_bits(n_cols);
  *n_buckets = ((int64_t)n_cols + ((int64_t)1 << *bits) - 1) >> *bits;
  *n_parts = (nnz + TP_PART - 1) / TP_PART;
}

int64_t transpose_scratch_bytes(int64_t n_rows, int64_t nnz, int32_t n_cols) {
  (void)n_rows;
  auto al = [](int64_t v) { return (v + 255) / 256 * 256; };
  if (nnz < PH_MIN_NNZ) return 0;
  int bits;
  int64_t n_buckets, n_parts;
  tp_geometry(nnz, n_cols, &bits, &n_buckets, &n_parts);
  if (n_buckets < 1 || n_buckets > TP_MAX_BUCKETS) return 0;
  return al((n_parts + 1) * 8) + al(n_parts * TP_PART * 2 + 64) + al(n_parts * TP_PART * 2 + 64) + al(n_parts * TP_PART * 4 + 64) + al((n_parts + 1) * 8) +
         al((n_buckets + 1) * n_parts * 2) + al(n_buckets * 8) + al((n_buckets + 1) * 4);
}

hipError_t launch_transpose_partitioned(hipStream_t st, int64_t n_rows, const int64_t* row_ptr, const int32_t* col_idx, int64_t nnz, int32_t n_cols,
                                        const int64_t* col_ptr, int32_t* cursor, int32_t* out_row_idx, int32_t col_lo, int32_t col_hi, char* scratch) {
  int bits;
  int64_t n_buckets, n_parts;
  auto al = [](int64_t v) { return (v + 255) / 256 * 256; };
  tp_geometry(nnz, n_cols, &bits, &n_buckets, &n_parts);
  if (n_buckets < 1 || n_buckets > TP_MAX_BUCKETS) return hipErrorInvalidValue;
  int64_t* R = reinterpret_cast<int64_t*>(scratch); scratch += al((n_parts + 1) * 8);
  unsigned short* bk_col = reinterpret_cast<unsigned short*>(scratch); scratch += al(n_parts * TP_PART * 2 + 64);
  unsigned short* bk_row16 = reinterpret_cast<unsigned short*>(scratch); scratch += al(n_parts * TP_PART * 2 + 64);
  int32_t* bk_row = reinterpret_cast<int32_t*>(scratch); scratch += al(n_parts * TP_PART * 4 + 64);
  int64_t* part_base = reinterpret_cast<int64_t*>(scratch); scratch += al((n_parts + 1) * 8);
  unsigned short* loc_t = reinterpret_cast<unsigned short*>(scratch); scratch += al((n_buckets + 1) * n_parts * 2);
  long long* weight = reinterpret_cast<long long*>(scratch); scratch += al(n_buckets * 8);
  int32_t* blk_prefix = reinterpret_cast<int32_t*>(scratch);
  const int vec_ok = (reinterpret_cast<uintptr_t>(col_idx) & 15) == 0;
  hipLaunchKernelGGL(tr_parts_kernel, dim3((unsigned)((n_parts + 256) / 256)), dim3(256), 0, st, n_rows, row_ptr, n_parts, R);
  hipLaunchKernelGGL(tp_partition_kernel, dim3((unsigned)n_parts), dim3(TP_THREADS), 0, st, n_rows, row_ptr, col_idx, R, bits, (int)n_buckets, n_parts, col_lo, col_hi, bk_col,
                     bk_row16, bk_row, part_base, loc_t, vec_ok);
  hipError_t we = launch_slice_weights(st, loc_t, (int)n_buckets, n_parts, weight);
  if (we != hipSuccess) return we;
  hipLaunchKernelGGL(tp_blockmap_kernel, dim3(1), dim3(SCAN_THREADS), 0, st, weight, (int)n_buckets, n_parts, blk_prefix);
  const int64_t max_blocks = n_buckets + nnz / TR_CHUNK;
  hipLaunchKernelGGL(tp_place_kernel, dim3((unsigned)max_blocks), dim3(TPP_THREADS), 0, st, bk_col, bk_row16, bk_row, part_base, loc_t, bits, (int)n_buckets, n_parts, blk_prefix, col_ptr, n_cols, cursor,
                     out_row_idx);
  return hipGetLastError();
}

__global__ __launch_bounds__(256) void row_work_csr_kernel(int64_t n_rows, const int64_t* __restrict__ a_rp, const int32_t* __restrict__ a_ci,
                                                           const int64_t* __restrict__ b_rp, int g_log2, unsigned long long* __restrict__ work) {
  const int G = 1 << g_log2;
  const int gl = threadIdx.x & (G - 1);
  const int64_t groups_per_block = 256 >> g_log2;
  for (int64_t r = (int64_t)blockIdx.x * groups_per_block + (threadIdx.x >> g_log2); r < n_rows;
       r += (int64_t)gridDim.x * groups_per_block) {
    const unsigned long long d = (unsigned long long)(b_rp[r + 1] - b_rp[r]);
    if (d == 0ull) continue;
    const int64_t s = a_rp[r], e = a_rp[r + 1];
    for (int64_t p = s + gl; p < e; p += G) atomicAdd(&work[a_ci[p]], d);
  }
}
hipError_t launch_row_work_csr(hipStream_t st, int n_cu, int64_t n_rows, const int64_t* a_row_ptr, const int32_t* a_col_idx,
                               const int64_t* b_row_ptr, int g_log2, int32_t n_items_a, int64_t* work) {
  hipError_t e = hipMemsetAsync(work, 0, sizeof(int64_t) * (size_t)n_items_a, st);
  if (e != hipSuccess || n_rows == 0) return e;
  const int64_t gpb = 256 >> g_log2;
  int64_t blocks = (n_rows + gpb - 1) / gpb;
  const int64_t cap = (int64_t)n_cu * 8;
  if (blocks > cap) blocks = cap;
  hipLaunchKernelGGL(row_work_csr_kernel, dim3((unsigned)blocks), dim3(256), 0, st, n_rows, a_row_ptr, a_col_idx, b_row_ptr, g_log2,
                     reinterpret_cast<unsigned long long*>(work));
  return hipGetLastError();
}


}
```

universal-recommender_amd/csrc/urcco_api.hip:

```cpp
#include <memory>

#include "urcco_internal.h"

using namespace urcco_detail;

#include <signal.h>
#include <unistd.h>

#include <mutex>

namespace urcco_detail {
char* err_buf() {
  static thread_local char buf[512] = "";
  return buf;
}

const DebugCfg& debug_cfg() {
  static const DebugCfg cfg = [] {
    DebugCfg c;
    const char* m = getenv("URCCO_DEBUG_MARKS");
    const char* p = getenv("URCCO_DEBUG_POISON");
    c.marks = m && *m && *m != '0';
    c.poison = p && *p && *p != '0';
    return c;
// ... 147 lines not shown
  (void)hipSetDevice(s->device);
  (void)hipStreamSynchronize(s->stream);
  debug_unregister(s);
  if (s->arena) (void)hipFree(s->arena);
  if (s->xlx_tab) (void)hipFree(s->xlx_tab);
  if (s->xlx_hi) (void)hipFree(s->xlx_hi);
  if (s->form_word) (void)hipFree(s->form_word);
  if (s->g_counts) { (void)hipFree(s->g_counts); (void)hipFree(s->g_cand_key); (void)hipFree(s->g_cand_col); }
  s->collect();
  for (hipEvent_t e : s->free_events) (void)hipEventDestroy(e);
  if (s->own_stream) (void)hipStreamDestroy(s->stream);
  delete s;
}

int urcco_session_synchronize(urcco_session* s) {
  if (!s) return fail(URCCO_BAD_ARG, "session is NULL");
  HIPC(hipStreamSynchronize(s->stream));
  return URCCO_OK;
}

int urcco_session_set_debug(urcco_session* s, int32_t flags) {
  if (!s) return fail(URCCO_BAD_ARG, "session is NULL");
  s->debug = flags;
  return URCCO_OK;
}

int urcco_session_set_expand_test(urcco_session* s, int64_t limit, int64_t prefix_seed) {
  if (!s || limit < 0 || prefix_seed < 0) return fail(URCCO_BAD_ARG, "urcco_session_set_expand_test: bad argument");
  s->narrow_limit = limit == 0 ? urcco::NARROW_LIMIT : (unsigned long long)limit;
  s->prefix_seed = prefix_seed;
  return URCCO_OK;
}

int urcco_session_expand_form(urcco_session* s, int32_t* form_host) {
  if (!s || !form_host) return fail(URCCO_BAD_ARG, "urcco_session_expand_form: bad argument");
  if (!s->form_word || !s->form_valid) return fail(URCCO_BAD_ARG, "urcco_session_expand_form: no rows were built on this session");
  HIPC(hipMemcpyAsync(form_host, s->form_word, sizeof(int32_t), hipMemcpyDeviceToHost, s->stream));
  HIPC(hipStreamSynchronize(s->stream));
  return URCCO_OK;
}

int urcco_session_set_timing(urcco_session* s, int32_t enable) {
  if (!s) return fail(URCCO_BAD_ARG, "session is NULL");
  s->collect();
  s->timing = enable != 0;
  for (int i = 0; i < URCCO_N_STAGES; ++i) { s->acc_ms[i] = 0; s->acc_n[i] = 0; }
  return URCCO_OK;
}

int urcco_session_get_timings(urcco_session* s, double* ms, int64_t* launches) {
  if (!s || !ms || !launches) return fail(URCCO_BAD_ARG, "urcco_session_get_timings: bad argument");
  s->collect();
  for (int i = 0; i < URCCO_N_STAGES; ++i) { ms[i] = s->acc_ms[i]; launches[i] = s->acc_n[i]; }
  return URCCO_OK;
}

int64_t urcco_session_scratch_bytes(const urcco_session* s) {
  if (!s) return 0;
  return (int64_t)s->arena_cap + (int64_t)s->g_cap * 16;
}

int urcco_dev_column_counts(urcco_session* s, int64_t nnz, const int32_t* col_idx, int32_t n_cols, int32_t* counts) {
  if (!s || nnz < 0 || n_cols < 0 || (nnz > 0 && !col_idx) || (n_cols > 0 && !counts)) return fail(URCCO_BAD_ARG, "urcco_dev_column_counts: bad argument");
  if (n_cols == 0) return URCCO_OK;
  const int64_t ph_bytes = urcco::column_counts_scratch_bytes(nnz, n_cols);
  if (ph_bytes > 0) URC(s->reserve((size_t)ph_bytes));
  s->begin(URCCO_STAGE_COLUMN_COUNTS);
  if (ph_bytes > 0)
    HIPC(urcco::launch_column_counts_partitioned(s->stream, col_idx, nnz, nullptr, n_cols, counts, s->take<char>((size_t)ph_bytes)));
  else
    HIPC(urcco::launch_column_counts(s->stream, s->n_cu, col_idx, nnz, n_cols, counts));
  s->end();
  return URCCO_OK;
}

int urcco_dev_downsample(urcco_session* s, int64_t n_rows, const int64_t* row_ptr, const int32_t* col_idx, int64_t nnz, int32_t n_cols,
                         const int32_t* raw_counts, int32_t seed, int32_t max_elements_per_row, int32_t row_rate_mode, int64_t row_base,
                         int64_t* out_row_ptr, int32_t* out_col_idx, int32_t* post_counts) {
  if (!s || n_rows < 0 || nnz < 0 || n_cols < 0 || !row_ptr || !out_row_ptr || (nnz > 0 && (!col_idx || !raw_counts || !out_col_idx)))
    return fail(URCCO_BAD_ARG, "urcco_dev_downsample: bad argument");
  if (max_elements_per_row <= 0) return fail(URCCO_BAD_ARG, "maxElementsPerRow must be positive, got %d", max_elements_per_row);
  if ((row_rate_mode & ~URCCO_RNG_MIX32) != URCCO_ROW_RATE_MAHOUT_INT_DIV && (row_rate_mode & ~URCCO_RNG_MIX32) != URCCO_ROW_RATE_FRACTIONAL)
    return fail(URCCO_BAD_ARG, "unknown row_rate_mode %d", row_rate_mode);
  if (post_counts && n_cols > 0) HIPC(hipMemsetAsync(post_counts, 0, sizeof(int32_t) * (size_t)n_cols, s->stream));
  if (nnz == 0) {
    HIPC(hipMemsetAsync(out_row_ptr, 0, sizeof(int64_t) * (size_t)(n_rows + 1), s->stream));
    return URCCO_OK;
  }
  const int64_t ph_bytes = post_counts ? urcco::column_counts_scratch_bytes(nnz, n_cols) : 0;
  const int64_t ds_tiles = (nnz + urcco::DS_TILE - 1) / urcco::DS_TILE;
  const size_t n_words = (size_t)ds_tiles * (urcco::DS_TILE / 64);
  const size_t thr_words = (size_t)n_cols + (size_t)n_cols / 8 + 2;
  URC(s->reserve(urcco_session::need(thr_words, 8) + urcco_session::need((size_t)ds_tiles + 1, 8) * 2 + urcco_session::need(n_words, 8) +
                 (size_t)ph_bytes + 256));
  unsigned long long* thresholds = s->take<unsigned long long>(thr_words);
  int64_t* tile_rows = s->take<int64_t>((size_t)ds_tiles + 1);
  int64_t* tile_count = s->take<int64_t>((size_t)ds_tiles + 1);
  unsigned long long* flags = s->take<unsigned long long>(n_words);
  s->begin(URCCO_STAGE_DOWNSAMPLE_FLAGS);
  HIPC(urcco::launch_downsample_flags(s->stream, s->n_cu, n_rows, row_ptr, col_idx, nnz, n_cols, raw_counts, thresholds, (uint32_t)seed,
                                      max_elements_per_row, row_rate_mode, row_base, tile_rows, flags, tile_count,
                                      ph_bytes > 0 ? nullptr : post_counts));
  s->end();
  s->begin(URCCO_STAGE_DOWNSAMPLE_SCAN);
  HIPC(urcco::launch_downsample_scan(s->stream, nnz, tile_count));
  s->end();
  s->begin(URCCO_STAGE_DOWNSAMPLE_COMPACT);
  HIPC(urcco::launch_downsample_compact(s->stream, n_rows, row_ptr, col_idx, nnz, tile_rows, flags, tile_count, out_row_ptr, out_col_idx));
  s->end();
  if (ph_bytes > 0) {
    s->begin(URCCO_STAGE_COLUMN_COUNTS);
    HIPC(urcco::launch_column_counts_partitioned(s->stream, out_col_idx, nnz, out_row_ptr + n_rows, n_cols, post_counts, s->take<char>((size_t)ph_bytes)));
    s->end();
  }
  return URCCO_OK;
}

int urcco_dev_transpose(urcco_session* s, int64_t n_rows, const int64_t* row_ptr, const int32_t* col_idx, int64_t nnz, int32_t n_cols,
                        const int32_t* counts, int32_t col_lo, int32_t col_hi, int64_t* out_col_ptr, int32_t* out_row_idx) {
  if (!s || n_rows < 0 || nnz < 0 || n_cols < 0 || !row_ptr || !out_col_ptr || (n_cols > 0 && !counts) || (nnz > 0 && (!col_idx || !out_row_idx)) ||
      col_lo < 0 || col_hi < col_lo || col_hi > n_cols)
    return fail(URCCO_BAD_ARG, "urcco_dev_transpose: bad argument");
  const int64_t n_tiles = ((int64_t)n_cols + urcco::SCAN_TILE - 1) / urcco::SCAN_TILE;
  const int64_t tr_bytes = urcco::transpose_scratch_bytes(n_rows, nnz, n_cols);
  URC(s->reserve(urcco_session::need((size_t)n_cols, 4) + urcco_session::need((size_t)n_tiles + 2, 8) + (size_t)tr_bytes + 256));
  int32_t* cursor = s->take<int32_t>((size_t)n_cols);
  int64_t* tile_sums = s->take<int64_t>((size_t)n_tiles + 2);
  s->begin(URCCO_STAGE_TRANSPOSE);
  HIPC(urcco::launch_scan_i32_range(s->stream, counts, n_cols, col_lo, col_hi, out_col_ptr, tile_sums));
  if (nnz > 0 && n_rows > 0) {
    int g = ceil_log2_i64((nnz + n_rows - 1) / n_rows);
    if (g < 1) g = 1;
    if (g > 6) g = 6;
    HIPC(hipMemsetAsync(cursor, 0, sizeof(int32_t) * (size_t)n_cols, s->stream));
    if (tr_bytes > 0) {
      HIPC(urcco::launch_transpose_partitioned(s->stream, n_rows, row_ptr, col_idx, nnz, n_cols, out_col_ptr, cursor, out_row_idx, col_lo, col_hi,
                                               s->take<char>((size_t)tr_bytes)));
    } else {
      HIPC(urcco::launch_transpose(s->stream, s->n_cu, n_rows, row_ptr, col_idx, g, out_col_ptr, cursor, out_row_idx, col_lo, col_hi));
    }
  }
  s->end();
  return URCCO_OK;
}

int urcco_dev_row_work_csr(urcco_session* s, int64_t n_rows, const int64_t* a_row_ptr, const int32_t* a_col_idx, int64_t nnz_a, const int64_t* b_row_ptr,
                           int32_t n_items_a, int64_t* work) {
  if (!s || n_rows < 0 || nnz_a < 0 || n_items_a < 0 || !a_row_ptr || !b_row_ptr || (nnz_a > 0 && !a_col_idx) || (n_items_a > 0 && !work))
    return fail(URCCO_BAD_ARG, "urcco_dev_row_work_csr: bad argument");
  int g = n_rows > 0 ? ceil_log2_i64((nnz_a + n_rows - 1) / n_rows) : 1;
  if (g < 1) g = 1;
  if (g > 6) g = 6;
  s->begin(URCCO_STAGE_ROW_WORK);
  HIPC(urcco::launch_row_work_csr(s->stream, s->n_cu, n_rows, a_row_ptr, a_col_idx, b_row_ptr, g, n_items_a, work));
  s->end();
  return URCCO_OK;
}

int urcco_dev_row_work(urcco_session* s, int32_t item_lo, int32_t item_hi, int32_t n_items_a, const int64_t* a_col_ptr, const int32_t* a_row_idx,
                       int64_t nnz_a_bound, const int64_t* b_row_ptr, int64_t* work) {
  if (!s || item_lo < 0 || item_hi < item_lo || item_hi > n_items_a || nnz_a_bound < 0 || !a_col_ptr || !b_row_ptr || (item_hi > item_lo && !work))
    return fail(URCCO_BAD_ARG, "urcco_dev_row_work: bad argument");
  const int64_t cap = nnz_a_bound;
  const int64_t n_tiles = (cap + urcco::SCAN_TILE - 1) / urcco::SCAN_TILE;
  URC(s->reserve(urcco_session::need((size_t)cap, 4) + urcco_session::need((size_t)cap + 1, 8) + urcco_session::need((size_t)n_tiles + 2, 8)));
  if (!s->form_word) HIPC(hipMalloc((void**)&s->form_word, sizeof(int32_t)));
  s->form_valid = false;
  int32_t* plen = s->take<int32_t>((size_t)cap);
  int64_t* wp = s->take<int64_t>((size_t)cap + 1);
  int64_t* tile_sums = s->take<int64_t>((size_t)n_tiles + 2);
  int32_t* form = s->form_word;
  s->begin(URCCO_STAGE_ROW_WORK);
  HIPC(urcco::launch_expand_prepare(s->stream, s->n_cu, a_col_ptr, n_items_a, a_row_idx, b_row_ptr, nullptr, 0, cap, nullptr, nullptr, plen, wp, tile_sums,
                                    urcco::ExpandForm{form, nullptr, 0, 0, s->narrow_limit, s->prefix_seed}));
  HIPC(urcco::launch_row_work(s->stream, s->n_cu, item_lo, item_hi, a_col_ptr, wp, tile_sums, form, work));
  s->form_valid = true;
  s->end();
  return URCCO_OK;
}

int urcco_dev_partition(urcco_session* s, int32_t n_items, const int64_t* work, int32_t n_parts, int32_t* bounds_host) {
  if (!s || n_items < 0 || n_parts <= 0 || n_parts > 4096 || !bounds_host || (n_items > 0 && !work)) return fail(URCCO_BAD_ARG, "urcco_dev_partition: bad argument");
  int32_t* bounds = nullptr;
  URC(urcco_detail::partition_dev(s, n_items, work, n_parts, nullptr, &bounds));
  HIPC(hipMemcpyAsync(bounds_host, bounds, sizeof(int32_t) * (size_t)(n_parts + 1), hipMemcpyDeviceToHost, s->stream));
  HIPC(hipStreamSynchronize(s->stream));
  return URCCO_OK;
}

int urcco_dev_merge_fragments(urcco_session* s, int32_t world, int32_t item_lo, int32_t item_hi, int32_t n_items, const void* lens, int32_t wire16,
                              const int32_t* entries, int64_t n_entries, const int64_t* sizes, const int32_t* counts, int64_t* out_col_ptr,
                              int32_t* out_row_idx) {
  if (!s || world <= 0 || item_lo < 0 || item_hi < item_lo || item_hi > n_items || n_entries < 0 || !sizes || !out_col_ptr || (n_items > 0 && !counts) ||
      (item_hi > item_lo && !lens) || (n_entries > 0 && (!entries || !out_row_idx)))
    return fail(URCCO_BAD_ARG, "urcco_dev_merge_fragments: bad argument");
  const int32_t n_range = item_hi - item_lo;
  const int64_t n_runs = (int64_t)world * n_range;
  const int64_t t_items = ((int64_t)n_items + urcco::SCAN_TILE - 1) / urcco::SCAN_TILE, t_runs = (n_runs + urcco::SCAN_TILE - 1) / urcco::SCAN_TILE;
  URC(s->reserve(urcco_session::need((size_t)n_runs + 1, 8) + urcco_session::need((size_t)(t_items > t_runs ? t_items : t_runs) + 2, 8)));
  int64_t* src_off = s->take<int64_t>((size_t)n_runs + 1);
  int64_t* tile_sums = s->take<int64_t>((size_t)(t_items > t_runs ? t_items : t_runs) + 2);
  s->begin(URCCO_STAGE_TRANSPOSE);
  HIPC(urcco::launch_scan_i32_range(s->stream, counts, n_items, item_lo, item_hi, out_col_ptr, tile_sums));
  if (wire16) {
    HIPC(urcco::launch_scan_u16(s->stream, static_cast<const unsigned short*>(lens), n_runs, src_off, tile_sums));
  } else {
    HIPC(urcco::launch_scan_i32(s->stream, static_cast<const int32_t*>(lens), n_runs, src_off, tile_sums));
  }
  HIPC(urcco::launch_frag_place(s->stream, s->n_cu, world, item_lo, n_range, lens, wire16, src_off, entries, out_col_ptr, sizes, out_row_idx));
  s->end();
  return URCCO_OK;
}

int urcco_dev_cco_rows(urcco_session* s, int32_t item_lo, int32_t item_hi, int32_t n_items_a, const int64_t* a_col_ptr,
                       const int32_t* a_row_idx, int64_t nnz_a_bound, const int64_t* b_row_ptr, const int32_t* b_col_idx, int32_t n_cols_b,
                       const int32_t* counts_a, const int32_t* counts_b, int64_t n_users, int32_t exclude_self, int32_t k,
                       int32_t has_min_llr, double min_llr, int32_t* out_count, int32_t* out_idx, double* out_llr, int64_t* stats_dev) {
  return urcco_detail::cco_rows_impl(s, item_lo, item_hi, n_items_a, a_col_ptr, a_row_idx, nnz_a_bound, b_row_ptr, b_col_idx, n_cols_b, counts_a, counts_b, n_users,
                                     exclude_self, k, has_min_llr, min_llr, out_count, out_idx, out_llr, stats_dev, nullptr, nullptr);
}

int urcco_dev_pack_counts(urcco_session* s, int64_t n_rows_b, const int64_t* b_row_ptr, const int32_t* b_col_idx, int64_t nnz_b_bound, const int32_t* counts_b,
                          int32_t n_cols_b, int32_t* out_packed, int32_t* out_bad) {
  return urcco_detail::pack_counts(s, b_row_ptr, n_rows_b, b_col_idx, nnz_b_bound, counts_b, n_cols_b, out_packed, out_bad);
}

int urcco_dev_cco_rows_packed(urcco_session* s, int32_t item_lo, int32_t item_hi, int32_t n_items_a, const int64_t* a_col_ptr,
                              const int32_t* a_row_idx, int64_t nnz_a_bound, const int64_t* b_row_ptr, const int32_t* b_col_idx, int32_t n_cols_b,
                              const int32_t* counts_a, const int32_t* counts_b, int64_t n_users, int32_t exclude_self, int32_t k,
                              int32_t has_min_llr, double min_llr, int32_t* out_count, int32_t* out_idx, double* out_llr, int64_t* stats_dev,
                              const int32_t* b_packed, const int32_t* pack_bad) {
  if ((b_packed == nullptr) != (pack_bad == nullptr)) return fail(URCCO_BAD_ARG, "urcco_dev_cco_rows_packed: b_packed and pack_bad come together");
  return urcco_detail::cco_rows_impl(s, item_lo, item_hi, n_items_a, a_col_ptr, a_row_idx, nnz_a_bound, b_row_ptr, b_col_idx, n_cols_b, counts_a, counts_b, n_users,
                                     exclude_self, k, has_min_llr, min_llr, out_count, out_idx, out_llr, stats_dev, nullptr, nullptr, nullptr, b_packed, pack_bad);
}

}

namespace urcco_detail {

int partition_dev(urcco_session* s, int32_t n_items, const int64_t* work, int32_t n_parts, int32_t* bounds_dev, int32_t** bounds_out) {
  const int64_t n_tiles = ((int64_t)n_items + urcco::SCAN_TILE - 1) / urcco::SCAN_TILE;
  URC(s->reserve(urcco_session::need((size_t)n_items + 1, 8) + urcco_session::need((size_t)n_tiles + 2, 8) + urcco_session::need((size_t)n_parts + 1, 4)));
  int64_t* prefix = s->take<int64_t>((size_t)n_items + 1);
  int64_t* tile_sums = s->take<int64_t>((size_t)n_tiles + 2);
  int32_t* bounds = bounds_dev ? bounds_dev : s->take<int32_t>((size_t)n_parts + 1);
  HIPC(urcco::launch_scan_i64(s->stream, work, n_items, prefix, tile_sums));
  HIPC(urcco::launch_partition(s->stream, n_items, prefix, n_parts, bounds));
  if (bounds_out) *bounds_out = bounds;
  return URCCO_OK;
}

int cco_rows_impl(urcco_session* s, int32_t item_lo, int32_t item_hi, int32_t n_items_a, const int64_t* a_col_ptr, const int32_t* a_row_idx, int64_t nnz_a_bound,
                  const int64_t* b_row_ptr, const int32_t* b_col_idx, int32_t n_cols_b, const int32_t* counts_a, const int32_t* counts_b, int64_t n_users,
                  int32_t exclude_self, int32_t k, int32_t has_min_llr, double min_llr, int32_t* out_count, int32_t* out_idx, double* out_llr, int64_t* stats_dev,
                  const unsigned* pre_pstart, const int32_t* pre_plen, int64_t* pre_tile_sums, const int32_t* b_packed, const int32_t* pack_bad, bool pk_known, int64_t b_nnz_bound) {
  if (!s || item_lo < 0 || item_hi < item_lo || item_hi > n_items_a || n_cols_b < 0 || n_users < 0 || nnz_a_bound < 0 || !a_col_ptr || !b_row_ptr)
    return fail(URCCO_BAD_ARG, "urcco_dev_cco_rows: bad argument");
  if (k <= 0) return fail(URCCO_BAD_ARG, "maxInterestingElements must be positive, got %d", k);
  const int32_t n = item_hi - item_lo;
  if (n == 0) {
    if (stats_dev) HIPC(hipMemsetAsync(stats_dev, 0, sizeof(int64_t) * URCCO_STATS_LEN, s->stream));
    return URCCO_OK;
  }
  if (!out_count || !out_idx || !out_llr || !counts_a || (n_cols_b > 0 && !counts_b)) return fail(URCCO_BAD_ARG, "urcco_dev_cco_rows: NULL buffer");
  HIPC(hipMemsetAsync(out_count, 0, sizeof(int32_t) * (size_t)n, s->stream));
  if (n_cols_b == 0 || n_users == 0) {
    if (stats_dev) HIPC(hipMemsetAsync(stats_dev, 0, sizeof(int64_t) * URCCO_STATS_LEN, s->stream));
    return URCCO_OK;
  }
  int key_bits = 1;
  while (((int64_t)1 << key_bits) <= (int64_t)n_cols_b) ++key_bits;
  const int count_bits = 32 - key_bits;
  if (count_bits < 1) return fail(URCCO_BAD_ARG, "n_cols_b %d too large for the packed accumulator", n_cols_b);
  const bool dense_bin6 = k > urcco::MP_KMAX_HOST || 3ll * k + 5 > 32768ll;
  if (dense_bin6) URC(s->ensure_global_bin(n_cols_b));
  if (!s->xlx_tab) {
    HIPC(hipMalloc((void**)&s->xlx_tab, sizeof(double) * urcco::XLX_TABLE_HOST));
    HIPC(urcco::launch_xlx_table(s->stream, s->xlx_tab));
  }
  if (!s->xlx_hi) HIPC(hipMalloc((void**)&s->xlx_hi, sizeof(double) * 2 * urcco::XLX_TABLE_HOST));
  if (s->xlx_hi_n != n_users) {
    HIPC(urcco::launch_xlx_hi_table(s->stream, s->xlx_hi, s->xlx_tab, n_users));
    s->xlx_hi_n = n_users;
  }
  const int64_t n_tiles = ((int64_t)n + urcco::BIN_TILE - 1) / urcco::BIN_TILE;
  const int64_t cap = nnz_a_bound;
  const int64_t p_tiles = (cap + urcco::SCAN_TILE - 1) / urcco::SCAN_TILE;
  if (!s->form_word) HIPC(hipMalloc((void**)&s->form_word, sizeof(int32_t)));
  s->form_valid = false;
  URC(s->reserve(urcco_session::need((size_t)cap, 8) + urcco_session::need((size_t)cap, 4) + (pre_pstart ? 0 : urcco_session::need((size_t)cap, 4)) + urcco_session::need((size_t)cap + 1, 8) +
                 urcco_session::need((size_t)p_tiles + 2, 8) +
                 urcco_session::need((size_t)n, 8) + urcco_session::need((size_t)(n_tiles + 1) * urcco::BIN_COLS_HOST, 8) +
                 urcco_session::need(urcco::BIN_OFF_LEN, 4) + urcco_session::need((size_t)n, 4) + urcco_session::need((size_t)n_items_a, 8) +
                 urcco_session::need((size_t)n_cols_b, 2) + urcco_session::need(1, 4) + urcco_session::need(urcco::CAND_SLOTS, 8) + urcco_session::need(1, 8) + urcco_session::need(URCCO_STATS_LEN, 8) +
                 urcco_session::need((size_t)n_users + 1, 4)));
  int64_t* pstart64 = s->take<int64_t>((size_t)cap);
  unsigned* own_pstart = pre_pstart ? nullptr : s->take<unsigned>((size_t)cap);
  int32_t* own_plen = s->take<int32_t>((size_t)cap);
  const unsigned* pstart32 = pre_pstart ? pre_pstart : own_pstart;
  int64_t* wp = s->take<int64_t>((size_t)cap + 1);
  int32_t* form = s->form_word;
  int64_t* p_tile_sums = s->take<int64_t>((size_t)p_tiles + 2);
  int64_t* work = s->take<int64_t>((size_t)n);
  int64_t* tile_counts = s->take<int64_t>((size_t)(n_tiles + 1) * urcco::BIN_COLS_HOST);
  int32_t* bin_off = s->take<int32_t>(urcco::BIN_OFF_LEN);
  int32_t* bin_rows = s->take<int32_t>((size_t)n);
  double* ent_a = s->take<double>((size_t)n_items_a);
  unsigned short* cnt_b16 = s->take<unsigned short>((size_t)n_cols_b);
  int32_t* cnt16_bad = s->take<int32_t>(1);
  unsigned long long* cand = s->take<unsigned long long>(urcco::CAND_SLOTS);
  double* xlx_n = s->take<double>(1);
  int64_t* stats = stats_dev ? stats_dev : s->take<int64_t>(URCCO_STATS_LEN);
  unsigned* b_rp32 = s->take<unsigned>((size_t)n_users + 1);

  const int32_t* packed = pk_known ? b_col_idx : ((b_packed && pack_bad && !(s->debug & urcco::DBG_UNPACKED_COUNTS)) ? b_packed : nullptr);
  const bool host_wide = packed == nullptr || (s->debug & urcco::DBG_ROW_KERNELS) != 0;
  const bool narrow_known = pk_known && !host_wide && b_nnz_bound >= 0 && b_nnz_bound < ((int64_t)1 << 32) &&
                            (unsigned long long)n_cols_b * (unsigned long long)urcco::SCAN_TILE < s->narrow_limit;
  const urcco::ExpandForm ef{form, pk_known ? nullptr : pack_bad, host_wide ? 1 : 0, narrow_known ? 1 : 0, s->narrow_limit, s->prefix_seed};
  int64_t* tile_sums = (pre_pstart && pre_plen && pre_tile_sums) ? pre_tile_sums : p_tile_sums;
  s->begin(URCCO_STAGE_ROW_WORK);
  if (pre_pstart && pre_plen)
    HIPC(urcco::launch_expand_scan(s->stream, a_col_ptr, n_items_a, pre_plen, cap, wp, tile_sums, pre_tile_sums != nullptr, pre_pstart, pstart64, ef));
  else
    HIPC(urcco::launch_expand_prepare(s->stream, s->n_cu, a_col_ptr, n_items_a, a_row_idx, b_row_ptr, b_rp32, n_users, cap, own_pstart, pstart64, own_plen, wp, tile_sums, ef));
  HIPC(urcco::launch_row_work(s->stream, s->n_cu, item_lo, item_hi, a_col_ptr, wp, tile_sums, form, work));
  s->form_valid = true;
  s->end();
  s->begin(URCCO_STAGE_BINNING);
  HIPC(hipMemsetAsync(stats, 0, sizeof(int64_t) * URCCO_STATS_LEN, s->stream));
  HIPC(urcco::launch_binning(s->stream, item_lo, n, work, counts_a, n_cols_b, count_bits, k, tile_counts, bin_off, bin_rows, stats));
  s->end();
  s->begin(URCCO_STAGE_ENTROPY);
  HIPC(urcco::launch_item_entropy(s->stream, counts_a, n_items_a, n_users, ent_a, xlx_n));
  HIPC(urcco::launch_narrow_counts(s->stream, s->n_cu, counts_b, n_cols_b, cnt_b16, cnt16_bad));
  s->end();

  urcco::CcoArgs a;
  a.bin_rows = bin_rows; a.bin_off = bin_off;
  a.a_col_ptr = a_col_ptr; a.pstart32 = pstart32; a.pstart64 = pstart64; a.wp = wp; a.form = form; a.work = work; a.b_col_idx = b_col_idx;
  a.b_packed = packed; a.pk_known = narrow_known ? 1 : 0;
  a.b_col_mask = pk_known ? (key_bits >= 32 ? 0xffffffffu : (1u << key_bits) - 1u) : 0xffffffffu;
  a.cnt_a = counts_a; a.cnt_b = counts_b; a.ent_a = ent_a; a.cnt_b16 = cnt_b16; a.cnt16_bad = cnt16_bad; a.xlx_n = xlx_n; a.xlx_tab = s->xlx_tab; a.xlx_hi = s->xlx_hi; a.col_ent = s->xlx_hi + urcco::XLX_TABLE_HOST; a.debug = s->debug;
  a.n_users = n_users; a.n_cols_b = n_cols_b; a.item_lo = item_lo; a.exclude_self = exclude_self ? 1 : 0; a.k = k;
  a.has_min_llr = has_min_llr ? 1 : 0; a.min_llr = min_llr; a.count_bits = count_bits;
  a.col_bytes = n_cols_b <= (1 << 8) ? 1 : (n_cols_b <= (1 << 16) ? 2 : (n_cols_b <= (1 << 24) ? 3 : 4));
  a.unordered = s->unordered_rows ? 1 : 0;
  a.g_log2 = 4;
  a.out_count = out_count; a.out_idx = out_idx; a.out_llr = out_llr;
  a.err = reinterpret_cast<unsigned long long*>(stats + 1 + 4 * urcco::NBINS);
  a.cand = s->timing ? cand : nullptr;
  if (s->timing) HIPC(hipMemsetAsync(cand, 0, sizeof(unsigned long long) * urcco::CAND_SLOTS, s->stream));
  a.g_counts = s->g_counts; a.g_cand_key = s->g_cand_key; a.g_cand_col = s->g_cand_col; a.g_blocks = dense_bin6 ? s->g_blocks : 0;
  for (int step = 0; step < urcco::NBINS; ++step) {
    const int bin = urcco::NBINS - 1 - step;
    s->begin(URCCO_STAGE_CCO_BIN0 + bin);
    HIPC(urcco::launch_cco_rows_bin(s->stream, s->n_cu, a, bin, n));
    s->end();
  }
  if (s->timing) HIPC(urcco::launch_bin_out_stats(s->stream, bin_rows, bin_off, item_lo, out_count, cand, stats));
  return URCCO_OK;
}

int pack_counts(urcco_session* s, const int64_t* b_row_ptr, int64_t n_rows_b, const int32_t* b_col_idx, int64_t nnz_bound, const int32_t* counts_b, int32_t n_cols_b,
                int32_t* out, int32_t* bad) {
  if (!s || !b_row_ptr || n_rows_b < 0 || nnz_bound < 0 || !out || !bad || (nnz_bound > 0 && (!b_col_idx || !counts_b))) return fail(URCCO_BAD_ARG, "pack_counts: bad argument");
  int key_bits = 1;
  while (((int64_t)1 << key_bits) <= (int64_t)n_cols_b) ++key_bits;
  const int count_bits = 32 - key_bits;
  if (count_bits < 1) return fail(URCCO_BAD_ARG, "n_cols_b %d too large for the packed accumulator", n_cols_b);
  URC(s->reserve(urcco_session::need((size_t)n_cols_b + 8, 2) + urcco_session::need(1, 4) + 256));
  unsigned short* c16 = s->take<unsigned short>((size_t)n_cols_b + 8);
  int32_t* bad16 = s->take<int32_t>(1);
  s->begin(URCCO_STAGE_ENTROPY);
  HIPC(urcco::launch_narrow_counts(s->stream, s->n_cu, counts_b, n_cols_b, c16, bad16));
  HIPC(urcco::launch_pack_counts(s->stream, s->n_cu, b_col_idx, b_row_ptr + n_rows_b, nnz_bound, c16, bad16, count_bits, out, bad));
  s->end();
  return URCCO_OK;
}

int expand_multi(urcco_session* s, int n, const int64_t* a_col_ptr, int32_t n_items_a, const int32_t* a_row_idx, int64_t cap, const int64_t* const* b_row_ptr,
                 int64_t n_users, unsigned* const* pstart, int32_t* const* plen, int64_t* const* tile_sums) {
  if (!s || n < 1 || n > urcco::EXPAND_MULTI_MAX || !a_col_ptr || cap < 0) return fail(URCCO_BAD_ARG, "expand_multi: bad argument");
  URC(s->reserve(urcco_session::need(((size_t)n_users + 2) * (size_t)n, 4) + 256));
  void* T = s->take<unsigned>(((size_t)n_users + 2) * (size_t)n);
  s->begin(URCCO_STAGE_ROW_WORK);
  HIPC(urcco::launch_expand_prepare_multi(s->stream, s->n_cu, a_col_ptr, n_items_a, a_row_idx, n, b_row_ptr, n_users, cap, pstart, plen, T, tile_sums));
  s->end();
  return URCCO_OK;
}

}

extern "C" {

int urcco_dev_compact_indicators(urcco_session* s, int32_t n_rows, int32_t k, const int32_t* count, const int32_t* idx, const double* llr,
                                 int64_t* out_row_ptr, int32_t* out_col_idx, double* out_llr) {
  if (!s || n_rows < 0 || k <= 0 || !out_row_ptr || (n_rows > 0 && (!count || !idx || !llr || !out_col_idx || !out_llr)))
    return fail(URCCO_BAD_ARG, "urcco_dev_compact_indicators: bad argument");
  const int64_t n_tiles = ((int64_t)n_rows + urcco::SCAN_TILE - 1) / urcco::SCAN_TILE;
  URC(s->reserve(urcco_session::need((size_t)n_tiles + 2, 8)));
  int64_t* tile_sums = s->take<int64_t>((size_t)n_tiles + 2);
  s->begin(URCCO_STAGE_COMPACT_INDICATORS);
  HIPC(urcco::launch_scan_i32(s->stream, count, n_rows, out_row_ptr, tile_sums));
  HIPC(urcco::launch_compact_indicators(s->stream, n_rows, k, count, idx, llr, out_row_ptr, out_col_idx, out_llr));
  s->end();
  return URCCO_OK;
}

struct urcco_key_table {
  urcco::KeyTable t{};
  int64_t capacity = 0;
  int device = 0;
};

void urcco_key_table_destroy(urcco_key_table* table) {
  if (!table) return;
  (void)hipSetDevice(table->device);
// ... 195 lines not shown
```

universal-recommender_amd/csrc/urcco_context.hip:

```cpp
#include <dlfcn.h>

#include <algorithm>
#include <atomic>
#include <chrono>
#include <condition_variable>
#include <functional>
#include <memory>
#include <future>
#include <mutex>
#include <string>
#include <thread>
#include <unordered_map>

#include "urcco_internal.h"

using namespace urcco_detail;

namespace {

struct Rccl {
  typedef struct { char internal[URCCO_UNIQUE_ID_BYTES]; } UniqueId;
  typedef void* Comm;
  void* handle = nullptr;
  int (*GetUniqueId)(UniqueId*) = nullptr;
// ... 401 lines not shown
    if (have_cb) {
      if (!cb.all_to_all_v) return fail(URCCO_BAD_ARG, "collectives.all_to_all_v is required (urcco.h, since 301)");
      return cb.all_to_all_v(cb.user, D.rank, send, soff, scnt, recv, roff, rcnt, (void*)st) == 0 ? URCCO_OK : fail(URCCO_RCCL_ERROR, "collectives.all_to_all_v failed");
    }
    RCCLC(rccl, rccl->GroupStart());
    for (int p = 0; p < world; ++p) {
      if (scnt[p] > 0) RCCLC(rccl, rccl->Send((const char*)send + soff[p], (size_t)scnt[p], Rccl::kInt8, p, D.comm, st));
      if (rcnt[p] > 0) RCCLC(rccl, rccl->Recv((char*)recv + roff[p], (size_t)rcnt[p], Rccl::kInt8, p, D.comm, st));
    }
    RCCLC(rccl, rccl->GroupEnd());
    return URCCO_OK;
  }
};

namespace {

int set_dev(const DevState& D) {
  HIPC(hipSetDevice(D.device));
  return URCCO_OK;
}
struct CallerDevice {
  int dev = -1;
  CallerDevice() { if (hipGetDevice(&dev) != hipSuccess) dev = -1; }
  ~CallerDevice() { if (dev >= 0) (void)hipSetDevice(dev); }
};

urcco_session* sess_of(urcco_context* c, DevState& D, int d) { return D.sessions[c->single_stream() ? 0 : (size_t)d]; }

int ensure_events(urcco_context* c, DevState& D, int n_ds) {
  URC(set_dev(D));
  while ((int)D.sessions.size() < n_ds) {
    urcco_session* s = nullptr;
    URC(urcco_session_create(D.device, c->emulate() ? (void*)c->emu_stream : nullptr, &s));
    s->debug = c->debug;
    s->timing = c->timing;
    s->unordered_rows = (c->flags & URCCO_FLAG_UNORDERED_ROWS) ? 1 : 0;
    D.sessions.push_back(s);
  }
  if ((int)D.ev.size() < n_ds) D.ev.resize((size_t)n_ds);
  for (int d = 0; d < n_ds; ++d) {
    EvState& E = D.ev[(size_t)d];
    E.s = sess_of(c, D, d);
    E.s->unordered_rows = (c->flags & URCCO_FLAG_UNORDERED_ROWS) ? 1 : 0;
    if (!E.ev_sampled) HIPC(hipEventCreateWithFlags(&E.ev_sampled, hipEventDisableTiming));
    if (!E.ev_done) HIPC(hipEventCreateWithFlags(&E.ev_done, hipEventDisableTiming));
    for (int q = 0; q < A_SETS; ++q)
      if (!E.ev_cons[q]) HIPC(hipEventCreateWithFlags(&E.ev_cons[q], hipEventDisableTiming));
    if (!E.ev_rp) HIPC(hipEventCreateWithFlags(&E.ev_rp, hipEventDisableTiming));
  }
  if (!D.a_ready) HIPC(hipEventCreateWithFlags(&D.a_ready, hipEventDisableTiming));
  if (!D.in_ready) HIPC(hipEventCreateWithFlags(&D.in_ready, hipEventDisableTiming));
  if (!D.b_expanded) HIPC(hipEventCreateWithFlags(&D.b_expanded, hipEventDisableTiming));
  if (!D.need_ready) HIPC(hipEventCreateWithFlags(&D.need_ready, hipEventDisableTiming));
  return URCCO_OK;
}

int stage_raw_counts(DevState& D, EvState& E, const Shard& sh, const DsParams& p) {
  URC(E.raw.ensure((size_t)p.n_cols + 1));
  return urcco_dev_column_counts(E.s, sh.nnz, sh.ci, (int32_t)p.n_cols, E.raw.p);
}
DBuf<int32_t>& post_of(DevState& D, int d) { return d == 0 ? D.a_post[D.par] : D.ev[(size_t)d].post; }

int stage_downsample(urcco_context* c, DevState& D, int d, const Shard& sh, const DsParams& p, int32_t seed) {
  EvState& E = D.ev[(size_t)d];
  URC(E.s_rp.ensure((size_t)sh.n_rows + 1));
  URC(E.s_ci.ensure((size_t)sh.nnz + 4));
  URC(post_of(D, d).ensure((size_t)p.n_cols + 1));
  return urcco_dev_downsample(E.s, sh.n_rows, sh.rp, sh.ci, sh.nnz, (int32_t)p.n_cols, E.raw.p, seed, p.max_rows, c->row_rate_mode, sh.row_base, E.s_rp.p,
                              E.s_ci.p, post_of(D, d).p);
}

int stage_rows(DevState& D, EvState& E, EvState& A, int d, const DsParams& pa, const DsParams& p, int64_t n_users, int64_t a_nnz_bound, bool pre_expanded = false) {
  const int32_t n = D.item_hi - D.item_lo;
  const size_t strided = (size_t)(n > 0 ? n : 1) * (size_t)p.k;
  URC(E.o_count.ensure((size_t)n + 1));
  URC(E.o_idx.ensure(strided));
  URC(E.o_llr.ensure(strided));
  URC(E.c_rp.ensure((size_t)n + 2));
  URC(E.c_idx.ensure(strided));
  URC(E.c_llr.ensure(strided));
  URC(E.stats.ensure(URCCO_STATS_LEN));
  if (!E.b_pk_known) {
    URC(E.b_pk.ensure((size_t)E.b_nnz_bound + 4));
    URC(E.pk_bad.ensure(1));
    URC(pack_counts(E.s, E.b_rp, E.b_rows, E.b_ci, E.b_nnz_bound, post_of(D, d).p, (int32_t)p.n_cols, E.b_pk.p, E.pk_bad.p));
  }
  URC(cco_rows_impl(E.s, D.item_lo, D.item_hi, (int32_t)pa.n_cols, D.a_cp[D.par].p, D.a_ri[D.par].p, a_nnz_bound, E.b_rp, E.b_ci, (int32_t)p.n_cols,
                    post_of(D, 0).p, post_of(D, d).p, n_users, d == 0 ? 1 : 0, p.k, p.has_min_llr, p.min_llr, E.o_count.p, E.o_idx.p, E.o_llr.p, E.stats.p,
                    pre_expanded ? E.pre_pstart.p : nullptr, pre_expanded ? E.pre_plen.p : nullptr, pre_expanded ? E.pre_tsum.p : nullptr,
                    E.b_pk_known ? nullptr : E.b_pk.p, E.b_pk_known ? nullptr : E.pk_bad.p, E.b_pk_known, E.b_nnz_bound));
  URC(urcco_dev_compact_indicators(E.s, n, p.k, E.o_count.p, E.o_idx.p, E.o_llr.p, E.c_rp.p, E.c_idx.p, E.c_llr.p));
  HIPC(hipEventRecord(E.ev_done, E.s->stream));
  HIPC(hipEventRecord(E.ev_cons[D.par], E.s->stream));
  E.cons_valid[D.par] = true;
  return URCCO_OK;
}

struct InputGate {
  const HostTrace* trace = nullptr;
  std::function<int(int)> after_chain;
  std::vector<int> order;
  std::vector<std::promise<int>> staged;
  std::vector<std::shared_future<int>> fut;
  std::vector<char> released;
  explicit InputGate(int n) : staged((size_t)n), fut((size_t)n), released((size_t)n, 0) {
    for (int d = 0; d < n; ++d) fut[(size_t)d] = staged[(size_t)d].get_future().share();
  }
  void release(int d, int status) {
    released[(size_t)d] = 1;
    staged[(size_t)d].set_value(status);
  }
  int wait(DevState& D, int d) {
    const int st = fut[(size_t)d].get();
    if (st != URCCO_OK) return fail(st, "dataset %d: staging failed", d);
    EvState& E = D.ev[(size_t)d];
    HIPC(hipStreamSynchronize(E.s->stream));
    const unsigned long long bad = E.h_verr ? *(volatile unsigned long long*)E.h_verr : 0ull;
    if (bad)
      return fail(URCCO_BAD_ARG, "dataset %d: %llu invalid entries (row_ptr not monotone, or col_idx out of [0, n_cols) / not strictly increasing inside a row)", d, bad);
    if (trace) trace->mark("matrices landed and checked", d);
    return URCCO_OK;
  }
};

int build_single(urcco_context* c, DevState& D, const std::vector<Shard>& sh, const std::vector<DsParams>& ps_, int64_t n_users, int32_t seed,
                 InputGate* gate) {
  const int n_ds = (int)sh.size();
  URC(set_dev(D));
  EvState& A = D.ev[0];
  D.item_lo = 0;
  D.item_hi = (int32_t)ps_[0].n_cols;
  URC(D.a_cp[D.par].ensure((size_t)ps_[0].n_cols + 2));
  URC(D.a_ri[D.par].ensure((size_t)sh[0].nnz + 4));
  std::atomic<bool> a_ok{false};
  const bool threaded = n_ds > 1 && !c->single_stream();
  std::promise<void> a_recorded;
  std::shared_future<void> a_recorded_f = a_recorded.get_future().share();
  bool fuse = n_ds >= 3 && n_ds - 1 <= urcco::EXPAND_MULTI_MAX && !(c->debug & urcco::DBG_UNFUSED_EXPAND) && gate == nullptr;
  for (int d = 1; d < n_ds; ++d) fuse = fuse && sh[(size_t)d].nnz < ((int64_t)1 << 32);
  const bool fold = fuse && n_ds <= urcco::EXPAND_MULTI_MAX && sh[0].nnz < ((int64_t)1 << 32);
  const int f0 = fold ? 0 : 1;
  std::vector<std::promise<int>> sampled((size_t)n_ds);
  std::vector<std::shared_future<int>> sampled_f((size_t)n_ds);
  for (int d = 0; d < n_ds; ++d) sampled_f[(size_t)d] = sampled[(size_t)d].get_future().share();
  std::promise<int> expanded;
  std::shared_future<int> expanded_f = expanded.get_future().share();
  const int64_t a_cap = sh[0].nnz;
  auto fused_expand = [&]() -> int {
    EvState& L = D.ev[1];
    if (L.s != A.s) HIPC(hipStreamWaitEvent(L.s->stream, D.a_ready, 0));
    std::vector<const int64_t*> rp((size_t)(n_ds - f0));
    std::vector<unsigned*> ps((size_t)(n_ds - f0));
    std::vector<int32_t*> pl((size_t)(n_ds - f0));
    std::vector<int64_t*> ts((size_t)(n_ds - f0));
    for (int d = f0; d < n_ds; ++d) {
      EvState& E = D.ev[(size_t)d];
      if (d > 0 && E.s != L.s) HIPC(hipStreamWaitEvent(L.s->stream, E.ev_sampled, 0));
      URC(E.pre_pstart.ensure((size_t)a_cap + 1));
      URC(E.pre_plen.ensure((size_t)a_cap + 1));
      URC(E.pre_tsum.ensure(expand_tile_words(a_cap)));
      ts[(size_t)(d - f0)] = E.pre_tsum.p;
      rp[(size_t)(d - f0)] = E.s_rp.p;
      ps[(size_t)(d - f0)] = E.pre_pstart.p;
      pl[(size_t)(d - f0)] = E.pre_plen.p;
    }
    URC(expand_multi(L.s, n_ds - f0, D.a_cp[D.par].p, (int32_t)ps_[0].n_cols, D.a_ri[D.par].p, a_cap, rp.data(), n_users, ps.data(), pl.data(), ts.data()));
    HIPC(hipEventRecord(D.b_expanded, L.s->stream));
    return URCCO_OK;
  };
  auto sample_secondary = [&](int d) -> int {
    URC(set_dev(D));
    EvState& E = D.ev[(size_t)d];
    if (gate) URC(gate->wait(D, d));
// ... 1326 lines not shown
```

universal-recommender_amd/csrc/urcco_internal.h:

```cpp
#pragma once
#include <hip/hip_runtime.h>

#include <cstdarg>
#include <cstdio>
#include <cstdlib>
#include <cstring>
#include <new>
#include <vector>

#include "../../include/urcco.h"
#include "cco_kernels.h"
static_assert(urcco::EXCH_SIZES == URCCO_EXCH_SIZES && urcco::STATS_LEN == URCCO_STATS_LEN, "include/urcco.h and cco_kernels.h agree");
static_assert(urcco::REC_MAX_CLAUSES == URCCO_REC_MAX_CLAUSES && urcco::REC_MAX_NUM == URCCO_REC_MAX_NUM && urcco::REC_NO_BACKFILL == URCCO_REC_NO_BACKFILL &&
                  urcco::REC_STATS_LEN == URCCO_REC_STATS_LEN && urcco::REC_MAX_RULES == URCCO_REC_MAX_RULES && urcco::REC_RULE_ANY == URCCO_RULE_ANY &&
                  urcco::REC_RULE_NONE == URCCO_RULE_NONE && urcco::REC_RULE_RANGE == URCCO_RULE_RANGE,
              "include/urcco.h and cco_kernels.h agree on the recommendation call");

struct urcco_session;
namespace urcco_detail {

char* err_buf();

inline int fail(int status, const char* fmt, ...) {
  va_list ap;
  va_start(ap, fmt);
  vsnprintf(err_buf(), 512, fmt, ap);
  va_end(ap);
  return status;
}

inline int hip_fail(hipError_t e, const char* what) {
  return fail(e == hipErrorOutOfMemory ? URCCO_OOM_DEVICE : URCCO_HIP_ERROR, "%s: %s", what, hipGetErrorString(e));
}

#define HIPC(expr)                                                  \
  do {                                                              \
    hipError_t _e = (expr);                                         \
    if (_e != hipSuccess) return urcco_detail::hip_fail(_e, #expr); \
  } while (0)

#define URC(expr)                  \
  do {                             \
    int _s = (expr);               \
    if (_s != URCCO_OK) return _s; \
  } while (0)

template <typename F>
inline int guarded(F&& body) {
  try {
    return body();
  } catch (const std::bad_alloc&) {
    return fail(URCCO_OOM_HOST, "out of host memory");
  } catch (const std::exception& e) {
    return fail(URCCO_INTERNAL, "unexpected exception: %s", e.what());
  } catch (...) {
    return fail(URCCO_INTERNAL, "unexpected exception");
  }
}

inline size_t align_up(size_t v, size_t a) { return (v + a - 1) / a * a; }

struct DebugCfg { bool marks = false, poison = false; };
const DebugCfg& debug_cfg();
void debug_mark(urcco_session* s, int which , int stage);
void debug_register(urcco_session* s);
void debug_unregister(urcco_session* s);
void debug_poison(void* p, size_t bytes, hipStream_t st, bool async);

inline int ceil_log2_i64(int64_t v) {
  int l = 0;
  while (((int64_t)1 << l) < v) ++l;
  return l;
}

}

namespace urcco_detail {
int cco_rows_impl(urcco_session* s, int32_t item_lo, int32_t item_hi, int32_t n_items_a, const int64_t* a_col_ptr, const int32_t* a_row_idx, int64_t nnz_a_bound,
                  const int64_t* b_row_ptr, const int32_t* b_col_idx, int32_t n_cols_b, const int32_t* counts_a, const int32_t* counts_b, int64_t n_users,
                  int32_t exclude_self, int32_t k, int32_t has_min_llr, double min_llr, int32_t* out_count, int32_t* out_idx, double* out_llr, int64_t* stats_dev,
                  const unsigned* pre_pstart, const int32_t* pre_plen, int64_t* pre_tile_sums = nullptr ,
                  const int32_t* b_packed = nullptr , const int32_t* pack_bad = nullptr ,
                  bool pk_known = false ,
                  int64_t b_nnz_bound = -1 );
int pack_counts(urcco_session* s, const int64_t* b_row_ptr, int64_t n_rows_b, const int32_t* b_col_idx, int64_t nnz_bound, const int32_t* counts_b, int32_t n_cols_b,
                int32_t* out, int32_t* bad);
int partition_dev(urcco_session* s, int32_t n_items, const int64_t* work, int32_t n_parts, int32_t* bounds_dev, int32_t** bounds_out);
int expand_multi(urcco_session* s, int n, const int64_t* a_col_ptr, int32_t n_items_a, const int32_t* a_row_idx, int64_t cap, const int64_t* const* b_row_ptr,
                 int64_t n_users, unsigned* const* pstart, int32_t* const* plen, int64_t* const* tile_sums = nullptr );
inline size_t expand_tile_words(int64_t cap) { return (size_t)((cap + urcco::SCAN_TILE - 1) / urcco::SCAN_TILE + 2); }
}

using namespace urcco_detail;

struct urcco_session {
  int device = 0;
  hipStream_t stream = nullptr;
  bool own_stream = false;
  int n_cu = 256;
  char* arena = nullptr;
  size_t arena_cap = 0;
  size_t arena_off = 0;
  int32_t* g_counts = nullptr;
  unsigned long long* g_cand_key = nullptr;
  int32_t* g_cand_col = nullptr;
  int64_t g_cols = 0;
  double* xlx_tab = nullptr;
  double* xlx_hi = nullptr;
  long long xlx_hi_n = -1;
  int debug = 0;
  unsigned long long narrow_limit = urcco::NARROW_LIMIT;
  long long prefix_seed = 0;
  int32_t* form_word = nullptr;
  bool form_valid = false;
  unsigned* marks = nullptr;
  unsigned mark_seq = 0;
  int unordered_rows = 0;
  bool timing = false;
  struct Rec { int stage; hipEvent_t e0, e1; };
  std::vector<Rec> recs;
  std::vector<hipEvent_t> free_events;
  double acc_ms[URCCO_N_STAGES] = {0};
  int64_t acc_n[URCCO_N_STAGES] = {0};

  hipEvent_t get_event() noexcept {
    if (!free_events.empty()) { hipEvent_t e = free_events.back(); free_events.pop_back(); return e; }
    hipEvent_t e = nullptr;
    (void)hipEventCreate(&e);
    return e;
  }
  void begin(int stage) noexcept {
    cur_stage = stage;
    if (marks) debug_mark(this, 0, stage);
    if (!timing) return;
    try {
      recs.reserve(recs.size() + 1);
      free_events.reserve(free_events.size() + 2 * (recs.size() + 1));
    } catch (...) {
      open_rec = false;
      return;
    }
    Rec r{stage, get_event(), get_event()};
    if (!r.e0 || !r.e1) { open_rec = false; return; }
    (void)hipEventRecord(r.e0, stream);
    recs.push_back(r);
    open_rec = true;
  }
  bool open_rec = false;
  int cur_stage = 0;
  void end() noexcept {
    if (marks) debug_mark(this, 1, cur_stage);
    if (!timing || !open_rec || recs.empty()) return;
    (void)hipEventRecord(recs.back().e1, stream);
    open_rec = false;
  }
  void collect() {
    (void)hipStreamSynchronize(stream);
    for (const Rec& r : recs) {
      float ms = 0.f;
      if (hipEventElapsedTime(&ms, r.e0, r.e1) == hipSuccess) { acc_ms[r.stage] += ms; acc_n[r.stage] += 1; }
      free_events.push_back(r.e0);
      free_events.push_back(r.e1);
    }
    recs.clear();
  }

  int reserve(size_t bytes) {
// ... 73 lines not shown
```

Before: 35.21 billion pairs/s.

## Fold memsets and blockmap launches into neighboring kernels to cut launch count

Removes several hipMemsetAsync calls and separate single-block launches. Weight arrays are now zeroed by the first block of the preceding kernel. The weights and blockmap kernels are merged with a last-block-done atomic counter. The expand form word is reset in-kernel through a fresh flag, and the pack/narrow-count work is folded into cco_rows_impl so it shares one verdict memset. The stats memset is replaced by zeroing the unused slots in the binning kernel. The aim is to reduce per-launch and per-memset overhead on the stream, at the cost of a threadfence/atomic last-block pattern and subtle ordering requirements for zero-initialization.

```diff
diff --git a/universal-recommender_amd/csrc/cco_common.h b/universal-recommender_amd/csrc/cco_common.h
--- a/universal-recommender_amd/csrc/cco_common.h
+++ b/universal-recommender_amd/csrc/cco_common.h
@@ -165,7 +165,7 @@
     if (over) s_over = 1;
     __syncthreads();
     if (threadIdx.x == 0) {
-      int f = form.host_narrow ? 0 : *form.word;
+      int f = (form.host_narrow || form.fresh) ? 0 : *form.word;
       if (form.host_narrow) s_over = 0;
       if (s_over) f |= FORM_TILE;
       if (form.pack_bad && *form.pack_bad != 0) f |= FORM_PACK;
diff --git a/universal-recommender_amd/csrc/cco_counts.hip b/universal-recommender_amd/csrc/cco_counts.hip
--- a/universal-recommender_amd/csrc/cco_counts.hip
+++ b/universal-recommender_amd/csrc/cco_counts.hip
@@ -270,7 +270,7 @@
 
 __global__ __launch_bounds__(PL_THREADS, 6) void pl_partition_kernel(const int32_t* __restrict__ ci, int64_t nnz_host, const int64_t* __restrict__ nnz_dev,
                                                                   int n_buckets, int64_t n_parts, unsigned short* __restrict__ bucketed,
-                                                                  unsigned short* __restrict__ loc_t, int vec_ok) {
+                                                                  unsigned short* __restrict__ loc_t, int vec_ok, long long* __restrict__ weight) {
   __shared__ int s_cnt[PL_COPIES * PL_MAX_BUCKETS];
   __shared__ uint4 s_stage4[PL_PART / 8];
   __shared__ long long s_wave[PL_THREADS / WAVE];
@@ -278,6 +278,8 @@
   const int64_t nnz = nnz_dev ? *nnz_dev : nnz_host;
   const int64_t e0 = (int64_t)blockIdx.x * PL_PART;
   const int64_t e1 = e0 + PL_PART < nnz ? e0 + PL_PART : nnz;
+  if (blockIdx.x == 0)
+    for (int b = threadIdx.x; b <= n_buckets; b += PL_THREADS) weight[b] = 0;
   if (e0 >= e1) {
     for (int b = threadIdx.x; b <= n_buckets; b += PL_THREADS) loc_t[(int64_t)b * n_parts + blockIdx.x] = 0;
     return;
@@ -417,39 +419,65 @@
   counts[j] = (int32_t)sum;
 }
 
-__global__ __launch_bounds__(256) void pl_weights_kernel(const unsigned short* __restrict__ loc_t, int64_t n_parts, unsigned long long* __restrict__ weight) {
-  __shared__ long long s_wave[256 / WAVE];
+enum { MAP_PL = 0, MAP_TP = 1 };
+__device__ __forceinline__ long long weight_of(long long* weight, int b) {
+  return (long long)atomicAdd(reinterpret_cast<unsigned long long*>(weight) + b, 0ull);
+}
+__global__ __launch_bounds__(SCAN_THREADS) void slice_blockmap_kernel(const unsigned short* __restrict__ loc_t, int n_buckets, int64_t n_parts, long long* weight,
+                                                                     int mode, long long S_or_chunk, int32_t* __restrict__ blk_prefix) {
+  static_assert(SCAN_THREADS == 256, "one block size for the sums and the map");
+  __shared__ long long s_wave[SCAN_THREADS / WAVE];
+  __shared__ long long s_total;
+  __shared__ int s_last;
   const unsigned short* lo_t = loc_t + (int64_t)blockIdx.x * n_parts;
   const unsigned short* hi_t = lo_t + n_parts;
   long long sum = 0;
   for (int64_t p = (int64_t)blockIdx.y * 256 + threadIdx.x; p < n_parts; p += (int64_t)gridDim.y * 256) sum += (long long)hi_t[p] - (long long)lo_t[p];
   long long tot;
   block_exclusive_scan<256>(sum, s_wave, &tot);
-  if (threadIdx.x == 0 && tot != 0) atomicAdd(&weight[blockIdx.x], (unsigned long long)tot);
-}
-__global__ __launch_bounds__(SCAN_THREADS) void pl_blockmap_kernel(const long long* __restrict__ weight, int n_buckets, int64_t n_parts, int S,
-                                                                  int32_t* __restrict__ blk_prefix) {
-  __shared__ long long s_wave[SCAN_THREADS / WAVE];
-  __shared__ long long s_total;
-  {
+  if (threadIdx.x == 0) {
+    if (tot != 0) atomicAdd(reinterpret_cast<unsigned long long*>(weight) + blockIdx.x, (unsigned long long)tot);
+    __threadfence();
+    const unsigned long long done = atomicAdd(reinterpret_cast<unsigned long long*>(weight) + n_buckets, 1ull);
+    s_last = done + 1ull == (unsigned long long)gridDim.x * gridDim.y;
+  }
+  __syncthreads();
+  if (!s_last) return;
+  __threadfence();
+  if (mode == MAP_PL) {
+    const int S = (int)S_or_chunk;
     const int b = threadIdx.x;
-    long long tot;
-    block_exclusive_scan(b < n_buckets ? weight[b] : 0ll, s_wave, &tot);
+    const long long w = b < n_buckets ? weight_of(weight, b) : 0ll;
+    block_exclusive_scan(w, s_wave, &tot);
     if (threadIdx.x == 0) s_total = tot;
-  }
-  __syncthreads();
-  const long long total = s_total;
-  const int b = threadIdx.x;
-  long long v = 0;
-  if (b < n_buckets) {
-    v = total > 0 ? (weight[b] * (long long)S * n_buckets + total - 1) / total : 1;
-    if (v < 1) v = 1;
-    if (v > n_parts) v = n_parts;
-  }
-  long long tot;
-  const long long ex = block_exclusive_scan(v, s_wave, &tot);
-  if (b < n_buckets) blk_prefix[b] = (int32_t)ex;
-  if (b == 0) blk_prefix[n_buckets] = (int32_t)tot;
+    __syncthreads();
+    const long long total = s_total;
+    long long v = 0;
+    if (b < n_buckets) {
+      v = total > 0 ? (w * (long long)S * n_buckets + total - 1) / total : 1;
+      if (v < 1) v = 1;
+      if (v > n_parts) v = n_parts;
+    }
+    const long long ex = block_exclusive_scan(v, s_wave, &tot);
+    if (b < n_buckets) blk_prefix[b] = (int32_t)ex;
+    if (b == 0) blk_prefix[n_buckets] = (int32_t)tot;
+  } else {
+    const long long chunk = S_or_chunk;
+    long long carry = 0;
+    for (int base = 0; base < n_buckets; base += SCAN_THREADS) {
+      const int b = base + threadIdx.x;
+      long long v = 0;
+      if (b < n_buckets) {
+        const long long w = weight_of(weight, b);
+        v = w > 0 ? (w + chunk - 1) / chunk : 1;
+        if (v > n_parts) v = n_parts;
+      }
+      const long long ex = block_exclusive_scan(v, s_wave, &tot);
+      if (b < n_buckets) blk_prefix[b] = (int32_t)(carry + ex);
+      carry += tot;
+    }
+    if (threadIdx.x == 0) blk_prefix[n_buckets] = (int32_t)carry;
+  }
 }
 
 constexpr int64_t PL_BLOCK_IDS = 49152;
@@ -471,11 +499,11 @@
   return pl_fits(n_cols);
 }
 
-hipError_t launch_slice_weights(hipStream_t st, const unsigned short* loc_t, int n_buckets, int64_t n_parts, long long* weight) {
-  hipError_t we = hipMemsetAsync(weight, 0, sizeof(long long) * (size_t)n_buckets, st);
-  if (we != hipSuccess) return we;
+hipError_t launch_slice_blockmap(hipStream_t st, const unsigned short* loc_t, int n_buckets, int64_t n_parts, long long* weight, bool transpose_map, long long S_or_chunk,
+                                 int32_t* blk_prefix) {
   const unsigned wsplit = (unsigned)(n_parts >= 8192 ? 8 : (n_parts >= 1024 ? 4 : 1));
-  hipLaunchKernelGGL(pl_weights_kernel, dim3((unsigned)n_buckets, wsplit), dim3(256), 0, st, loc_t, n_parts, reinterpret_cast<unsigned long long*>(weight));
+  hipLaunchKernelGGL(slice_blockmap_kernel, dim3((unsigned)n_buckets, wsplit), dim3(SCAN_THREADS), 0, st, loc_t, n_buckets, n_parts, weight,
+                     transpose_map ? (int)MAP_TP : (int)MAP_PL, S_or_chunk, blk_prefix);
   return hipGetLastError();
 }
 
@@ -486,7 +514,7 @@
   if (pl_fits(n_cols)) {
     const int64_t n_buckets = ((int64_t)n_cols + PL_BUCKET - 1) >> PL_BITS;
     const int64_t n_parts = (nnz + PL_PART - 1) / PL_PART;
-    need = al(n_parts * PL_PART * 2 + 64) + al((n_buckets + 1) * n_parts * 2) + al(n_buckets * 8) + al((n_buckets + 1) * 4) +
+    need = al(n_parts * PL_PART * 2 + 64) + al((n_buckets + 1) * n_parts * 2) + al((n_buckets + 1) * 8) + al((n_buckets + 1) * 4) +
            al(pl_max_blocks((int)n_buckets, pl_splits((int)n_buckets, n_parts, false)) * (int64_t)PL_BUCKET * 4);
   }
   if ((((int64_t)n_cols + PH_BUCKET - 1) >> PH_BITS) <= PH_MAX_BUCKETS) {
@@ -510,13 +538,12 @@
     const int S = pl_splits(n_buckets, n_parts);
     unsigned short* bucketed = reinterpret_cast<unsigned short*>(scratch); scratch += al(n_parts * PL_PART * 2 + 64);
     unsigned short* loc_t = reinterpret_cast<unsigned short*>(scratch); scratch += al(((int64_t)n_buckets + 1) * n_parts * 2);
-    long long* weight = reinterpret_cast<long long*>(scratch); scratch += al((int64_t)n_buckets * 8);
+    long long* weight = reinterpret_cast<long long*>(scratch); scratch += al(((int64_t)n_buckets + 1) * 8);
     int32_t* blk_prefix = reinterpret_cast<int32_t*>(scratch); scratch += al(((int64_t)n_buckets + 1) * 4);
     unsigned* partial = reinterpret_cast<unsigned*>(scratch);
-    hipLaunchKernelGGL(pl_partition_kernel, dim3((unsigned)n_parts), dim3(PL_THREADS), 0, st, col_idx, nnz, nnz_dev, n_buckets, n_parts, bucketed, loc_t, vec_ok);
-    hipError_t we = launch_slice_weights(st, loc_t, n_buckets, n_parts, weight);
+    hipLaunchKernelGGL(pl_partition_kernel, dim3((unsigned)n_parts), dim3(PL_THREADS), 0, st, col_idx, nnz, nnz_dev, n_buckets, n_parts, bucketed, loc_t, vec_ok, weight);
+    hipError_t we = launch_slice_blockmap(st, loc_t, n_buckets, n_parts, weight, false, S, blk_prefix);
     if (we != hipSuccess) return we;
-    hipLaunchKernelGGL(pl_blockmap_kernel, dim3(1), dim3(SCAN_THREADS), 0, st, weight, n_buckets, n_parts, S, blk_prefix);
     hipLaunchKernelGGL(pl_hist_kernel, dim3((unsigned)pl_max_blocks(n_buckets, S)), dim3(PLH_THREADS), 0, st, bucketed, loc_t, n_buckets, n_parts,
                        blk_prefix, n_cols, partial);
     hipLaunchKernelGGL(pl_reduce_kernel, dim3((unsigned)(((int64_t)n_cols + 255) / 256)), dim3(256), 0, st, partial, blk_prefix, n_cols, counts);
diff --git a/universal-recommender_amd/csrc/cco_expand.hip b/universal-recommender_amd/csrc/cco_expand.hip
--- a/universal-recommender_amd/csrc/cco_expand.hip
+++ b/universal-recommender_amd/csrc/cco_expand.hip
@@ -36,8 +36,8 @@
   }
   if (over) atomicAdd(bad, over);
 }
-hipError_t launch_narrow_counts(hipStream_t st, int n_cu, const int32_t* counts, int64_t n, unsigned short* out16, int32_t* bad) {
-  hipError_t e = hipMemsetAsync(bad, 0, sizeof(int32_t), st);
+hipError_t launch_narrow_counts(hipStream_t st, int n_cu, const int32_t* counts, int64_t n, unsigned short* out16, int32_t* bad, bool bad_is_zero) {
+  hipError_t e = bad_is_zero ? hipSuccess : hipMemsetAsync(bad, 0, sizeof(int32_t), st);
   if (e != hipSuccess || n <= 0) return e;
   int64_t blocks = (n + 255) / 256;
   if (blocks > (int64_t)n_cu * 8) blocks = (int64_t)n_cu * 8;
@@ -101,8 +101,8 @@
   if (n_bad) atomicAdd(bad, n_bad);
 }
 hipError_t launch_pack_counts(hipStream_t st, int n_cu, const int32_t* col_idx, const int64_t* nnz_dev, int64_t nnz_bound, const unsigned short* counts16,
-                              const int32_t* bad16, int32_t count_bits, int32_t* out, int32_t* bad) {
-  hipError_t e = hipMemsetAsync(bad, 0, sizeof(int32_t), st);
+                              const int32_t* bad16, int32_t count_bits, int32_t* out, int32_t* bad, bool bad_is_zero) {
+  hipError_t e = bad_is_zero ? hipSuccess : hipMemsetAsync(bad, 0, sizeof(int32_t), st);
   if (e != hipSuccess || nnz_bound <= 0) return e;
   const int shift = 32 - count_bits;
   int64_t blocks = (nnz_bound / 4 + 255) / 256;
@@ -411,8 +411,7 @@
 }
 hipError_t launch_expand_scan(hipStream_t st, const int64_t* a_col_ptr, int32_t n_items_a, const int32_t* plen, int64_t cap, int64_t* wp, int64_t* tile_sums,
                               bool tile_sums_ready, const unsigned* pstart32, int64_t* pstart64, ExpandForm form) {
-  hipError_t e = hipMemsetAsync(form.word, 0, sizeof(int32_t), st);
-  if (e != hipSuccess) return e;
+  form.fresh = 1;
   return expand_scan(st, plen, cap, wp, tile_sums, a_col_ptr + n_items_a, tile_sums_ready, pstart32, pstart64, form);
 }
 
diff --git a/universal-recommender_amd/csrc/cco_kernels.h b/universal-recommender_amd/csrc/cco_kernels.h
--- a/universal-recommender_amd/csrc/cco_kernels.h
+++ b/universal-recommender_amd/csrc/cco_kernels.h
@@ -43,6 +43,7 @@
   int32_t host_narrow;
   unsigned long long limit;
   long long seed;
+  int32_t fresh = 0;
 };
 
 struct CcoArgs {
@@ -97,7 +98,8 @@
                                             int32_t* counts, char* scratch);
 
 hipError_t launch_scan_i32(hipStream_t st, const int32_t* in, int64_t n, int64_t* out, int64_t* tile_sums);
-hipError_t launch_slice_weights(hipStream_t st, const unsigned short* loc_t, int n_buckets, int64_t n_parts, long long* weight);
+hipError_t launch_slice_blockmap(hipStream_t st, const unsigned short* loc_t, int n_buckets, int64_t n_parts, long long* weight, bool transpose_map, long long S_or_chunk,
+                                 int32_t* blk_prefix);
 
 hipError_t launch_downsample_flags(hipStream_t st, int n_cu, int64_t n_rows, const int64_t* row_ptr, const int32_t* col_idx, int64_t nnz,
                                    int32_t n_cols, const int32_t* raw_counts, unsigned long long* thresholds, uint32_t seed, int32_t max_n,
@@ -156,11 +158,11 @@
                              const int64_t* bounds, int32_t* counts);
 
 hipError_t launch_pack_counts(hipStream_t st, int n_cu, const int32_t* col_idx, const int64_t* nnz_dev, int64_t nnz_bound, const unsigned short* counts16,
-                              const int32_t* bad16, int32_t count_bits, int32_t* out, int32_t* bad);
+                              const int32_t* bad16, int32_t count_bits, int32_t* out, int32_t* bad, bool bad_is_zero = false );
 hipError_t launch_xlx_table(hipStream_t st, double* tab);
 hipError_t launch_xlx_hi_table(hipStream_t st, double* tab , const double* xlx_tab, long long n_users);
 hipError_t launch_item_entropy(hipStream_t st, const int32_t* counts, int32_t n, long long n_users, double* ent, double* xlx_n);
-hipError_t launch_narrow_counts(hipStream_t st, int n_cu, const int32_t* counts, int64_t n, unsigned short* out16, int32_t* bad);
+hipError_t launch_narrow_counts(hipStream_t st, int n_cu, const int32_t* counts, int64_t n, unsigned short* out16, int32_t* bad, bool bad_is_zero = false );
 
 hipError_t launch_expand_prepare(hipStream_t st, int n_cu, const int64_t* a_col_ptr, int32_t n_items_a, const int32_t* a_row_idx,
                                  const int64_t* b_row_ptr, unsigned* b_rp32_scratch , int64_t n_rows_b, int64_t cap,
diff --git a/universal-recommender_amd/csrc/cco_rows.hip b/universal-recommender_amd/csrc/cco_rows.hip
--- a/universal-recommender_amd/csrc/cco_rows.hip
+++ b/universal-recommender_amd/csrc/cco_rows.hip
@@ -154,6 +154,7 @@
         stats[1 + 2 * NBINS + k] = s_tot[IBINS + NBINS + k];
       }
       stats[0] = s_tot[IBINS + 2 * NBINS];
+      for (int w = 1 + 3 * NBINS; w < STATS_LEN - 1; ++w) stats[w] = 0;
       stats[STATS_LEN - 1] = s_tot[0] + s_tot[1];
     }
   }
diff --git a/universal-recommender_amd/csrc/cco_transpose.hip b/universal-recommender_amd/csrc/cco_transpose.hip
--- a/universal-recommender_amd/csrc/cco_transpose.hip
+++ b/universal-recommender_amd/csrc/cco_transpose.hip
@@ -43,7 +43,10 @@
 constexpr int TR_PART = 16384;
 constexpr int64_t TR_CHUNK = 1 << 18;
 
-__global__ __launch_bounds__(256) void tr_parts_kernel(int64_t n_rows, const int64_t* __restrict__ rp, int64_t n_parts, int64_t* __restrict__ R) {
+__global__ __launch_bounds__(256) void tr_parts_kernel(int64_t n_rows, const int64_t* __restrict__ rp, int64_t n_parts, int64_t* __restrict__ R,
+                                                       long long* __restrict__ weight, int n_buckets) {
+  if (blockIdx.x == 0)
+    for (int b = threadIdx.x; b <= n_buckets; b += 256) weight[b] = 0;
   const int64_t p = (int64_t)blockIdx.x * 256 + threadIdx.x;
   if (p > n_parts) return;
   if (p == n_parts) { R[p] = n_rows; return; }
@@ -246,23 +249,6 @@
   for (int v = threadIdx.x; v * 8 < n; v += TP_THREADS) dst[v] = s_stage4[v];
 }
 
-__global__ __launch_bounds__(SCAN_THREADS) void tp_blockmap_kernel(const long long* __restrict__ weight, int n_buckets, int64_t n_parts, int32_t* __restrict__ blk_prefix) {
-  __shared__ long long s_wave[SCAN_THREADS / WAVE];
-  long long carry = 0;
-  for (int base = 0; base < n_buckets; base += SCAN_THREADS) {
-    const int b = base + threadIdx.x;
-    long long v = 0;
-    if (b < n_buckets) {
-      v = weight[b] > 0 ? (weight[b] + TR_CHUNK - 1) / TR_CHUNK : 1;
-      if (v > n_parts) v = n_parts;
-    }
-    long long tot;
-    const long long ex = block_exclusive_scan(v, s_wave, &tot);
-    if (b < n_buckets) blk_prefix[b] = (int32_t)(carry + ex);
-    carry += tot;
-  }
-  if (threadIdx.x == 0) blk_prefix[n_buckets] = (int32_t)carry;
-}
 
 constexpr int TPP_THREADS = 1024;
 constexpr int TPP_LPS = 4;
@@ -361,7 +347,7 @@
   tp_geometry(nnz, n_cols, &bits, &n_buckets, &n_parts);
   if (n_buckets < 1 || n_buckets > TP_MAX_BUCKETS) return 0;
   return al((n_parts + 1) * 8) + al(n_parts * TP_PART * 2 + 64) + al(n_parts * TP_PART * 2 + 64) + al(n_parts * TP_PART * 4 + 64) + al((n_parts + 1) * 8) +
-         al((n_buckets + 1) * n_parts * 2) + al(n_buckets * 8) + al((n_buckets + 1) * 4);
+         al((n_buckets + 1) * n_parts * 2) + al((n_buckets + 1) * 8) + al((n_buckets + 1) * 4);
 }
 
 hipError_t launch_transpose_partitioned(hipStream_t st, int64_t n_rows, const int64_t* row_ptr, const int32_t* col_idx, int64_t nnz, int32_t n_cols,
@@ -377,15 +363,14 @@
   int32_t* bk_row = reinterpret_cast<int32_t*>(scratch); scratch += al(n_parts * TP_PART * 4 + 64);
   int64_t* part_base = reinterpret_cast<int64_t*>(scratch); scratch += al((n_parts + 1) * 8);
   unsigned short* loc_t = reinterpret_cast<unsigned short*>(scratch); scratch += al((n_buckets + 1) * n_parts * 2);
-  long long* weight = reinterpret_cast<long long*>(scratch); scratch += al(n_buckets * 8);
+  long long* weight = reinterpret_cast<long long*>(scratch); scratch += al((n_buckets + 1) * 8);
   int32_t* blk_prefix = reinterpret_cast<int32_t*>(scratch);
   const int vec_ok = (reinterpret_cast<uintptr_t>(col_idx) & 15) == 0;
-  hipLaunchKernelGGL(tr_parts_kernel, dim3((unsigned)((n_parts + 256) / 256)), dim3(256), 0, st, n_rows, row_ptr, n_parts, R);
+  hipLaunchKernelGGL(tr_parts_kernel, dim3((unsigned)((n_parts + 256) / 256)), dim3(256), 0, st, n_rows, row_ptr, n_parts, R, weight, (int)n_buckets);
   hipLaunchKernelGGL(tp_partition_kernel, dim3((unsigned)n_parts), dim3(TP_THREADS), 0, st, n_rows, row_ptr, col_idx, R, bits, (int)n_buckets, n_parts, col_lo, col_hi, bk_col,
                      bk_row16, bk_row, part_base, loc_t, vec_ok);
-  hipError_t we = launch_slice_weights(st, loc_t, (int)n_buckets, n_parts, weight);
+  hipError_t we = launch_slice_blockmap(st, loc_t, (int)n_buckets, n_parts, weight, true, TR_CHUNK, blk_prefix);
   if (we != hipSuccess) return we;
-  hipLaunchKernelGGL(tp_blockmap_kernel, dim3(1), dim3(SCAN_THREADS), 0, st, weight, (int)n_buckets, n_parts, blk_prefix);
   const int64_t max_blocks = n_buckets + nnz / TR_CHUNK;
   hipLaunchKernelGGL(tp_place_kernel, dim3((unsigned)max_blocks), dim3(TPP_THREADS), 0, st, bk_col, bk_row16, bk_row, part_base, loc_t, bits, (int)n_buckets, n_parts, blk_prefix, col_ptr, n_cols, cursor,
                      out_row_idx);
diff --git a/universal-recommender_amd/csrc/urcco_api.hip b/universal-recommender_amd/csrc/urcco_api.hip
--- a/universal-recommender_amd/csrc/urcco_api.hip
+++ b/universal-recommender_amd/csrc/urcco_api.hip
@@ -253,12 +253,12 @@
   if (max_elements_per_row <= 0) return fail(URCCO_BAD_ARG, "maxElementsPerRow must be positive, got %d", max_elements_per_row);
   if ((row_rate_mode & ~URCCO_RNG_MIX32) != URCCO_ROW_RATE_MAHOUT_INT_DIV && (row_rate_mode & ~URCCO_RNG_MIX32) != URCCO_ROW_RATE_FRACTIONAL)
     return fail(URCCO_BAD_ARG, "unknown row_rate_mode %d", row_rate_mode);
-  if (post_counts && n_cols > 0) HIPC(hipMemsetAsync(post_counts, 0, sizeof(int32_t) * (size_t)n_cols, s->stream));
+  const int64_t ph_bytes = (post_counts && nnz > 0) ? urcco::column_counts_scratch_bytes(nnz, n_cols) : 0;
+  if (post_counts && n_cols > 0 && ph_bytes == 0) HIPC(hipMemsetAsync(post_counts, 0, sizeof(int32_t) * (size_t)n_cols, s->stream));
   if (nnz == 0) {
     HIPC(hipMemsetAsync(out_row_ptr, 0, sizeof(int64_t) * (size_t)(n_rows + 1), s->stream));
     return URCCO_OK;
   }
-  const int64_t ph_bytes = post_counts ? urcco::column_counts_scratch_bytes(nnz, n_cols) : 0;
   const int64_t ds_tiles = (nnz + urcco::DS_TILE - 1) / urcco::DS_TILE;
   const size_t n_words = (size_t)ds_tiles * (urcco::DS_TILE / 64);
   const size_t thr_words = (size_t)n_cols + (size_t)n_cols / 8 + 2;
@@ -425,7 +425,8 @@
 int cco_rows_impl(urcco_session* s, int32_t item_lo, int32_t item_hi, int32_t n_items_a, const int64_t* a_col_ptr, const int32_t* a_row_idx, int64_t nnz_a_bound,
                   const int64_t* b_row_ptr, const int32_t* b_col_idx, int32_t n_cols_b, const int32_t* counts_a, const int32_t* counts_b, int64_t n_users,
                   int32_t exclude_self, int32_t k, int32_t has_min_llr, double min_llr, int32_t* out_count, int32_t* out_idx, double* out_llr, int64_t* stats_dev,
-                  const unsigned* pre_pstart, const int32_t* pre_plen, int64_t* pre_tile_sums, const int32_t* b_packed, const int32_t* pack_bad, bool pk_known, int64_t b_nnz_bound) {
+                  const unsigned* pre_pstart, const int32_t* pre_plen, int64_t* pre_tile_sums, const int32_t* b_packed, const int32_t* pack_bad, bool pk_known, int64_t b_nnz_bound,
+                  int32_t* pack_into, int32_t* pack_verdict, int64_t pack_rows_b) {
   if (!s || item_lo < 0 || item_hi < item_lo || item_hi > n_items_a || n_cols_b < 0 || n_users < 0 || nnz_a_bound < 0 || !a_col_ptr || !b_row_ptr)
     return fail(URCCO_BAD_ARG, "urcco_dev_cco_rows: bad argument");
   if (k <= 0) return fail(URCCO_BAD_ARG, "maxInterestingElements must be positive, got %d", k);
@@ -484,6 +485,17 @@
   double* xlx_n = s->take<double>(1);
   int64_t* stats = stats_dev ? stats_dev : s->take<int64_t>(URCCO_STATS_LEN);
   unsigned* b_rp32 = s->take<unsigned>((size_t)n_users + 1);
+  const bool pack_here = pack_into != nullptr && pack_verdict != nullptr && !pk_known && pack_rows_b >= 0 && b_nnz_bound >= 0;
+  if (pack_here) {
+    b_packed = pack_into;
+    pack_bad = pack_verdict;
+    cnt16_bad = pack_verdict + 1;
+    s->begin(URCCO_STAGE_ENTROPY);
+    HIPC(hipMemsetAsync(pack_verdict, 0, 2 * sizeof(int32_t), s->stream));
+    HIPC(urcco::launch_narrow_counts(s->stream, s->n_cu, counts_b, n_cols_b, cnt_b16, cnt16_bad, true));
+    HIPC(urcco::launch_pack_counts(s->stream, s->n_cu, b_col_idx, b_row_ptr + pack_rows_b, b_nnz_bound, cnt_b16, cnt16_bad, count_bits, pack_into, pack_verdict, true));
+    s->end();
+  }
 
   const int32_t* packed = pk_known ? b_col_idx : ((b_packed && pack_bad && !(s->debug & urcco::DBG_UNPACKED_COUNTS)) ? b_packed : nullptr);
   const bool host_wide = packed == nullptr || (s->debug & urcco::DBG_ROW_KERNELS) != 0;
@@ -500,12 +512,11 @@
   s->form_valid = true;
   s->end();
   s->begin(URCCO_STAGE_BINNING);
-  HIPC(hipMemsetAsync(stats, 0, sizeof(int64_t) * URCCO_STATS_LEN, s->stream));
   HIPC(urcco::launch_binning(s->stream, item_lo, n, work, counts_a, n_cols_b, count_bits, k, tile_counts, bin_off, bin_rows, stats));
   s->end();
   s->begin(URCCO_STAGE_ENTROPY);
   HIPC(urcco::launch_item_entropy(s->stream, counts_a, n_items_a, n_users, ent_a, xlx_n));
-  HIPC(urcco::launch_narrow_counts(s->stream, s->n_cu, counts_b, n_cols_b, cnt_b16, cnt16_bad));
+  if (!pack_here) HIPC(urcco::launch_narrow_counts(s->stream, s->n_cu, counts_b, n_cols_b, cnt_b16, cnt16_bad));
   s->end();
 
   urcco::CcoArgs a;
diff --git a/universal-recommender_amd/csrc/urcco_context.hip b/universal-recommender_amd/csrc/urcco_context.hip
--- a/universal-recommender_amd/csrc/urcco_context.hip
+++ b/universal-recommender_amd/csrc/urcco_context.hip
@@ -507,13 +507,12 @@
   URC(E.stats.ensure(URCCO_STATS_LEN));
   if (!E.b_pk_known) {
     URC(E.b_pk.ensure((size_t)E.b_nnz_bound + 4));
-    URC(E.pk_bad.ensure(1));
-    URC(pack_counts(E.s, E.b_rp, E.b_rows, E.b_ci, E.b_nnz_bound, post_of(D, d).p, (int32_t)p.n_cols, E.b_pk.p, E.pk_bad.p));
+    URC(E.pk_bad.ensure(2));
   }
   URC(cco_rows_impl(E.s, D.item_lo, D.item_hi, (int32_t)pa.n_cols, D.a_cp[D.par].p, D.a_ri[D.par].p, a_nnz_bound, E.b_rp, E.b_ci, (int32_t)p.n_cols,
                     post_of(D, 0).p, post_of(D, d).p, n_users, d == 0 ? 1 : 0, p.k, p.has_min_llr, p.min_llr, E.o_count.p, E.o_idx.p, E.o_llr.p, E.stats.p,
                     pre_expanded ? E.pre_pstart.p : nullptr, pre_expanded ? E.pre_plen.p : nullptr, pre_expanded ? E.pre_tsum.p : nullptr,
-                    E.b_pk_known ? nullptr : E.b_pk.p, E.b_pk_known ? nullptr : E.pk_bad.p, E.b_pk_known, E.b_nnz_bound));
+                    nullptr, nullptr, E.b_pk_known, E.b_nnz_bound, E.b_pk_known ? nullptr : E.b_pk.p, E.b_pk_known ? nullptr : E.pk_bad.p, E.b_rows));
   URC(urcco_dev_compact_indicators(E.s, n, p.k, E.o_count.p, E.o_idx.p, E.o_llr.p, E.c_rp.p, E.c_idx.p, E.c_llr.p));
   HIPC(hipEventRecord(E.ev_done, E.s->stream));
   HIPC(hipEventRecord(E.ev_cons[D.par], E.s->stream));
diff --git a/universal-recommender_amd/csrc/urcco_internal.h b/universal-recommender_amd/csrc/urcco_internal.h
--- a/universal-recommender_amd/csrc/urcco_internal.h
+++ b/universal-recommender_amd/csrc/urcco_internal.h
@@ -82,7 +82,10 @@
                   const unsigned* pre_pstart, const int32_t* pre_plen, int64_t* pre_tile_sums = nullptr ,
                   const int32_t* b_packed = nullptr , const int32_t* pack_bad = nullptr ,
                   bool pk_known = false ,
-                  int64_t b_nnz_bound = -1 );
+                  int64_t b_nnz_bound = -1 ,
+                  int32_t* pack_into = nullptr ,
+                  int32_t* pack_verdict = nullptr ,
+                  int64_t pack_rows_b = 0 );
 int pack_counts(urcco_session* s, const int64_t* b_row_ptr, int64_t n_rows_b, const int32_t* b_col_idx, int64_t nnz_bound, const int32_t* counts_b, int32_t n_cols_b,
                 int32_t* out, int32_t* bad);
 int partition_dev(urcco_session* s, int32_t n_items, const int64_t* work, int32_t n_parts, int32_t* bounds_dev, int32_t** bounds_out);
```

New measurement: 35.20 billion pairs/s. Within noise of the previous version (-0.0%).
